# jianzongwu/betrayed-by-captions

Hardware: AMD Instinct MI355X
Metric: images/sec (COCO-shaped 1024x1024, 100 queries, forward-only) (higher is better)
Workload: dtype f32; 1 GPU; configs[1]: R50 + 100 queries, 1024x1024, batch 2/GPU, forward-only; global_batch=2, parallelism=replicas x1, precision=fp32 (parity mode, f16x3 MFMA), hip_graph=True, x3_overflow=False, library_fallbacks=0

## Files before the change

### betrayed-by-captions_amd/csrc/x3s_gemm.hip

```cpp
#include <mutex>
#include "x3.h"

typedef __attribute__((address_space(3))) void* xs_lds_t;

struct XsConv {
  int H, W, C, OH, OW, KW, stride, pad, taps;
};

struct XsArgs {
  const void* A;
  int lda;
  int a_rpb;
  uint32_t a_bstride;
  CggX3W w;
  const float* bias;
  const void* res;
  int ldr, res_fmt, res_mod;
  void* out;
  int ldc, out_fmt;
  int M, N, K, relu, tiles_n, n_tiles32;
  XsConv cv;
  uint32_t a_bytes, w_bytes;
  int* flag;
};

template <int N>
__device__ __forceinline__ void xs_wait_vmcnt() {
  asm volatile("s_waitcnt vmcnt(%0)" ::"n"(N) : "memory");
}

__device__ __forceinline__ void xs_barrier() {
  asm volatile("" ::: "memory");
  __builtin_amdgcn_s_barrier();
  asm volatile("" ::: "memory");
}

#define XS_OOB 0xFFFFFF00u

struct XsTap {
  int c, c0, tap, ky, kx;
};

struct XsEpi {
  __amdgpu_buffer_rsrc_t orsrc, rrsrc;
  float lo_clamp;
  int mr0;
  int pb, y0, x0;
};

__device__ __forceinline__ uint32_t xs_sel(uint32_t a, uint32_t b, uint32_t mask) { return (b & mask) | (a & ~mask); }

__device__ __forceinline__ uint2 xs_pair_swap(const uint2 v) {
  uint2 r;
  r.x = cgg_lane_xor1(v.x);
  r.y = cgg_lane_xor1(v.y);
  return r;
}

__device__ __forceinline__ void xs_load_res(u32x4 (&rv)[4], const XsArgs& p, const __amdgpu_buffer_rsrc_t rrsrc, int& mres, int ncol0,
                                            int lane) {
  const int q = lane & 7;
  const bool cok = ncol0 + 4 * q < p.N;
  const uint32_t coff = (uint32_t)(ncol0 * 4 + 16 * q);
#pragma unroll
  for (int ps = 0; ps < 4; ++ps) {
    int mr = mres + 8 * ps;
    if (p.res_mod) {
      mr = mr >= p.res_mod ? mr - p.res_mod : mr;
      if (p.res_mod < 32) mr %= p.res_mod;
    }
    rv[ps] = __builtin_amdgcn_raw_buffer_load_b128(rrsrc, cok ? (uint32_t)(mr * p.ldr) * 4u + coff : XS_OOB, 0, 0);
  }
  mres += 32;
  if (p.res_mod) mres = p.res_mod >= 32 ? (mres >= p.res_mod ? mres - p.res_mod : mres) : mres % p.res_mod;
}

template <int RES, int OUT, int TW = 0>
__device__ __forceinline__ float xs_finish_column(const float* scratch, int TM_, const XsArgs& p, const XsEpi& e, int mrow0, int ncol0,
                                                  int lane, float amax, const u32x4 (&rv0)[4], bool have_rv0) {
  const int r8 = lane >> 3, q = lane & 7;
  const uint32_t om = 0u - (uint32_t)(q & 1);
  const bool cok = ncol0 + 4 * q < p.N;
  const uint32_t coff = (uint32_t)(ncol0 * 4 + 16 * q);
  int mres = e.mr0;
  auto load_res = [&](u32x4 (&rv)[4]) { xs_load_res(rv, p, e.rrsrc, mres, ncol0, lane); };
  u32x4 rv[4], rn[4];
  if (RES) {
    if (have_rv0) {
#pragma unroll
      for (int ps = 0; ps < 4; ++ps) rv[ps] = rv0[ps];
      mres += 32;
      if (p.res_mod) mres = p.res_mod >= 32 ? (mres >= p.res_mod ? mres - p.res_mod : mres) : mres % p.res_mod;
    } else {
      load_res(rv);
    }
  }
#pragma unroll 1
  for (int mt = 0; mt < TM_; ++mt) {
    const float* sc = scratch + mt * 1024;
    if (RES && mt + 1 < TM_) load_res(rn);
    f32x4 v[4];
#pragma unroll
    for (int ps = 0; ps < 4; ++ps) {
      const int rr = r8 + 8 * ps;
      v[ps] = *reinterpret_cast<const f32x4*>(sc + rr * 32 + (q ^ ((rr >> 1) & 1)) * 4);
    }
#pragma unroll
    for (int ps = 0; ps < 4; ++ps) {
      const int rr = r8 + 8 * ps;
      f32x4 w = v[ps];
      if (RES == 1) {
        w += __builtin_bit_cast(f32x4, rv[ps]) * CGG_X3_ASCALE;
      } else if (RES == 2) {
        const uint32_t r0 = rv[ps][0], r1 = rv[ps][1], r2 = rv[ps][2], r3 = rv[ps][3];
        const uint2 keep = {xs_sel(r0, r2, om), xs_sel(r1, r3, om)};
        const uint2 send = {xs_sel(r2, r0, om), xs_sel(r3, r1, om)};
        const uint2 got = xs_pair_swap(send);
        const uint2 hh = {xs_sel(keep.x, got.x, om), xs_sel(keep.y, got.y, om)};
        const uint2 ll = {xs_sel(got.x, keep.x, om), xs_sel(got.y, keep.y, om)};
        const f32x2 h0 = __builtin_convertvector(__builtin_bit_cast(f16x2, hh.x), f32x2);
        const f32x2 h1 = __builtin_convertvector(__builtin_bit_cast(f16x2, hh.y), f32x2);
        const f32x2 l0 = __builtin_convertvector(__builtin_bit_cast(f16x2, ll.x), f32x2);
        const f32x2 l1 = __builtin_convertvector(__builtin_bit_cast(f16x2, ll.y), f32x2);
        w += f32x4{h0[0] + l0[0], h0[1] + l0[1], h1[0] + l1[0], h1[1] + l1[1]};
      }
#pragma unroll
      for (int k = 0; k < 4; ++k) w[k] = fmaxf(w[k], e.lo_clamp);
      uint32_t oo;
      if constexpr (TW > 0) {
        const int R = mrow0 + 32 * mt + rr, oy = e.y0 + R / TW, ox = e.x0 + R % TW;
        oo = (cok && oy < p.cv.H && ox < p.cv.W) ? (uint32_t)((e.pb + oy * p.cv.W + ox) * p.ldc) * 4u + coff : XS_OOB;
      } else {
        oo = cok ? (uint32_t)((mrow0 + 32 * mt + rr) * p.ldc) * 4u + coff : XS_OOB;
      }
      u32x4 o;
      if (OUT == 2) {
        const float wmax = __builtin_fmaxf(__builtin_fmaxf(fabsf(w[0]), fabsf(w[1])), __builtin_fmaxf(fabsf(w[2]), fabsf(w[3])));
        amax = __builtin_fmaxf(amax, (TW > 0 && oo == XS_OOB) ? 0.f : wmax);
        uint2 h, l;
        cgg_x3_split2(w[0], w[1], h.x, l.x);
        cgg_x3_split2(w[2], w[3], h.y, l.y);
        const uint2 got = xs_pair_swap(uint2{xs_sel(l.x, h.x, om), xs_sel(l.y, h.y, om)});
        o = u32x4{xs_sel(h.x, got.x, om), xs_sel(h.y, got.y, om), xs_sel(got.x, l.x, om), xs_sel(got.y, l.y, om)};
      } else {
        o = __builtin_bit_cast(u32x4, w * CGG_X3_INV_ASCALE);
      }
      __builtin_amdgcn_raw_buffer_store_b128(o, e.orsrc, oo, 0, 0);
    }
    if (RES) {
#pragma unroll
      for (int ps = 0; ps < 4; ++ps) rv[ps] = rn[ps];
    }
  }
  return amax;
}

__device__ __forceinline__ XsEpi xs_epi_setup(const XsArgs& p, int mrow0, int lane) {
  XsEpi e;
  e.orsrc = cgg_buffer_rsrc(p.out, (uint32_t)(((size_t)(p.M - 1) * p.ldc + p.N) * 4));
  const int res_rows = p.res_mod ? p.res_mod : p.M;
  e.rrsrc = cgg_buffer_rsrc(p.res_fmt ? p.res : p.out, p.res_fmt ? (uint32_t)(((size_t)(res_rows - 1) * p.ldr + p.N) * 4) : 0u);
  e.lo_clamp = p.relu ? 0.f : -__builtin_inff();
  e.mr0 = mrow0 + (lane >> 3);
  if (p.res_fmt && p.res_mod) e.mr0 %= p.res_mod;
  return e;
}

template <int TM, int TN, int TW = 0>
__device__ __forceinline__ float xs_epilogue(const f32x16 (&acc)[TM][TN], float* scratch, const XsArgs& p, const XsEpi& e, int mrow0,
                                             int ntile0, int lane, const u32x4 (&rv0)[4]) {
  const int j = lane & 31, hi5 = lane >> 5;
  const int fmt = p.res_fmt * 2 + (p.out_fmt - 1);
  float amax = 0.f;
#pragma unroll
  for (int nt = 0; nt < TN; ++nt) {
    const int ncol = (ntile0 + nt) * 32 + j;
    const bool nok = ncol < p.N;
    const float cs = nok ? p.w.scale[ncol] * CGG_X3_ASCALE : 0.f;
    const float bs = (nok && p.bias) ? p.bias[ncol] * CGG_X3_ASCALE : 0.f;
#pragma unroll
    for (int mt = 0; mt < TM; ++mt) {
#pragma unroll
      for (int r = 0; r < 16; ++r) {
        const int rr = (r & 3) + 8 * (r >> 2) + 4 * hi5;
        scratch[mt * 1024 + rr * 32 + (((j >> 2) ^ ((rr >> 1) & 1)) << 2) + (j & 3)] = acc[mt][nt][r] * cs + bs;
      }
    }
    const int ncol0 = (ntile0 + nt) * 32;
    if constexpr (TW > 0) {
      amax = fmt == 0 ? xs_finish_column<0, 1, TW>(scratch, TM, p, e, mrow0, ncol0, lane, amax, rv0, false)
                      : xs_finish_column<0, 2, TW>(scratch, TM, p, e, mrow0, ncol0, lane, amax, rv0, false);
    } else
    switch (fmt) {
      case 0: amax = xs_finish_column<0, 1>(scratch, TM, p, e, mrow0, ncol0, lane, amax, rv0, false); break;
      case 1: amax = xs_finish_column<0, 2>(scratch, TM, p, e, mrow0, ncol0, lane, amax, rv0, false); break;
      case 2: amax = xs_finish_column<1, 1>(scratch, TM, p, e, mrow0, ncol0, lane, amax, rv0, nt == 0); break;
      case 3: amax = xs_finish_column<1, 2>(scratch, TM, p, e, mrow0, ncol0, lane, amax, rv0, nt == 0); break;
      case 4: amax = xs_finish_column<2, 1>(scratch, TM, p, e, mrow0, ncol0, lane, amax, rv0, nt == 0); break;
      default: amax = xs_finish_column<2, 2>(scratch, TM, p, e, mrow0, ncol0, lane, amax, rv0, nt == 0); break;
    }
  }
  return amax;
}

template <int TM, int TN, int MT>
__device__ __forceinline__ void xs_compute_chunk(f32x16 (&acc)[TM][TN], const unsigned char* ab, const unsigned char* bb,
                                               const int (&aoffs)[2][2]) {
  u32x4 bh[2][TN], bl[2][TN], ah[2], al[2];
#pragma unroll
  for (int nt = 0; nt < TN; ++nt) {
    bh[0][nt] = *reinterpret_cast<const u32x4*>(bb + nt * 4096);
    bl[0][nt] = *reinterpret_cast<const u32x4*>(bb + nt * 4096 + 2048);
  }
  ah[0] = *reinterpret_cast<const u32x4*>(ab + aoffs[0][0]);
  al[0] = *reinterpret_cast<const u32x4*>(ab + aoffs[0][1]);
#pragma unroll
  for (int ks = 0; ks < 2; ++ks) {
#pragma unroll
    for (int mt = 0; mt < TM; ++mt) {
      const int cur = (ks * TM + mt) & 1, nxt = cur ^ 1;
      if (mt + 1 < TM) {
        ah[nxt] = *reinterpret_cast<const u32x4*>(ab + (mt + 1) * MT + aoffs[ks][0]);
        al[nxt] = *reinterpret_cast<const u32x4*>(ab + (mt + 1) * MT + aoffs[ks][1]);
      } else if (ks == 0) {
        ah[nxt] = *reinterpret_cast<const u32x4*>(ab + aoffs[1][0]);
        al[nxt] = *reinterpret_cast<const u32x4*>(ab + aoffs[1][1]);
      }
      if (ks == 0 && mt == (TM > 1 ? TM - 2 : 0)) {
#pragma unroll
        for (int nt = 0; nt < TN; ++nt) {
          bh[1][nt] = *reinterpret_cast<const u32x4*>(bb + nt * 4096 + 1024);
          bl[1][nt] = *reinterpret_cast<const u32x4*>(bb + nt * 4096 + 2048 + 1024);
        }
      }
      __builtin_amdgcn_sched_barrier(0);
#pragma unroll
      for (int nt = 0; nt < TN; ++nt)
        acc[mt][nt] = __builtin_amdgcn_mfma_f32_32x32x16_f16(__builtin_bit_cast(f16x8, al[cur]), __builtin_bit_cast(f16x8, bh[ks][nt]),
                                                             acc[mt][nt], 0, 0, 0);
#pragma unroll
      for (int nt = 0; nt < TN; ++nt)
        acc[mt][nt] = __builtin_amdgcn_mfma_f32_32x32x16_f16(__builtin_bit_cast(f16x8, ah[cur]), __builtin_bit_cast(f16x8, bl[ks][nt]),
                                                             acc[mt][nt], 0, 0, 0);
#pragma unroll
      for (int nt = 0; nt < TN; ++nt)
        acc[mt][nt] = __builtin_amdgcn_mfma_f32_32x32x16_f16(__builtin_bit_cast(f16x8, ah[cur]), __builtin_bit_cast(f16x8, bh[ks][nt]),
                                                             acc[mt][nt], 0, 0, 0);
    }
  }
}

template <bool CONV, int TM, int TN, int WM, int WN, int KG, int SA, int SB>
__global__ __launch_bounds__(64 * WM * WN * KG) void cgg_gemm_x3s_kernel(const XsArgs p) {
  constexpr int NWG = WM * WN, NW = NWG * KG, BM = 32 * TM * WM, BN = 32 * TN * WN;
  constexpr int A_SLOT = KG * BM * 128, B_SLOT = KG * BN * 128;
  constexpr int NA = BM / 8 / NWG, NB = BN / 8 / NWG;
  constexpr int DA = SA - 1, DB = SB - 1;
  constexpr int LDS = SA * A_SLOT + SB * B_SLOT;
  static_assert(BM % (8 * NWG) == 0 && BN % (8 * NWG) == 0, "tile rows / columns must split evenly over the waves' DMA pieces");
  static_assert(SA >= SB && SB >= 2, "A runs at least as far ahead as B");
  static_assert(LDS >= NWG * TM * 4096 + (KG - 1) * NWG * TM * TN * 4096, "LDS: the rings must cover the reduce buffer + epilogue scratch");
  static_assert(KG == 1 || KG == 2, "one or two k-groups");
  constexpr int WAIT = (DA > DB ? NA : 0) + (DB - 1) * (NA + NB);
  extern __shared__ __attribute__((aligned(16))) unsigned char xs_smem[];
  const int tid = threadIdx.x, lane = tid & 63;
  const int wave = __builtin_amdgcn_readfirstlane(tid >> 6);
  const int j = lane & 31, hi5 = lane >> 5;
  const int kg = wave / NWG, wg = wave - kg * NWG;
  const int wm = wg / WN, wn = wg - wm * WN;
  const int bid = cgg_xcd_remap(blockIdx.x, gridDim.x);
  const int tile_m = bid / p.tiles_n, tile_n = bid - tile_m * p.tiles_n;
  const int m0 = tile_m * BM, nt0 = tile_n * (BN / 32);
  const int KS = p.K >> 4, nchunk = p.K >> 5;
  const int niter = (nchunk + KG - 1) / KG;

  const __amdgpu_buffer_rsrc_t arsrc = cgg_buffer_rsrc(p.A, p.a_bytes);
  uint32_t arow[NA];
  uint32_t amask[NA];
  int ag[NA];
#pragma unroll
  for (int i = 0; i < NA; ++i) {
    const int q = wave + NW * i;
    ag[i] = KG == 1 ? 0 : q / (BM / 8);
    const int r = (q - ag[i] * (BM / 8)) * 8 + (lane >> 3);
    const int u = (lane & 7) ^ ((r >> 1) & 7);
    const int m = m0 + r;
    const int mc = m < p.M ? m : p.M - 1;
    if constexpr (CONV) {
      const int ohw = p.cv.OH * p.cv.OW;
      const int b = mc / ohw, rr = mc - b * ohw;
      const int oy = rr / p.cv.OW, ox = rr - oy * p.cv.OW;
      const int iy0 = oy * p.cv.stride - p.cv.pad, ix0 = ox * p.cv.stride - p.cv.pad;
      arow[i] = (uint32_t)(((b * p.cv.H + iy0) * p.cv.W + ix0) * p.cv.C) * 4u + 16u * u;
      uint32_t mk = 0;
      const int KH = p.cv.taps / p.cv.KW;
      for (int ky = 0; ky < KH; ++ky)
        for (int kx = 0; kx < p.cv.KW; ++kx) {
          const int iy = iy0 + ky, ix = ix0 + kx;
          if (iy >= 0 && iy < p.cv.H && ix >= 0 && ix < p.cv.W) mk |= 1u << (ky * p.cv.KW + kx);
        }
      amask[i] = mk;
    } else {
      if (p.a_rpb > 0) {
        const int b = mc / p.a_rpb;
        arow[i] = ((uint32_t)b * p.a_bstride + (uint32_t)(mc - b * p.a_rpb) * (uint32_t)p.lda) * 4u + 16u * u;
      } else {
        arow[i] = (uint32_t)mc * (uint32_t)p.lda * 4u + 16u * u;
      }
      amask[i] = 0;
    }
  }
  const __amdgpu_buffer_rsrc_t brsrc = cgg_buffer_rsrc(p.w.hi, p.w_bytes);
  uint32_t boff[NB];
  int bg[NB];
#pragma unroll
  for (int i = 0; i < NB; ++i) {
    const int q = wave + NW * i;
    bg[i] = KG == 1 ? 0 : q / (BN / 8);
    const int b = q - bg[i] * (BN / 8);
    const int nt = b >> 2, piece = (b >> 1) & 1, ks = b & 1;
    const int ntc = nt0 + nt < p.n_tiles32 ? nt0 + nt : p.n_tiles32 - 1;
    boff[i] = (uint32_t)(((piece * p.n_tiles32 + ntc) * KS + ks) * 64 + lane) * 16u;
  }

  XsTap at[KG];
#pragma unroll
  for (int g = 0; g < KG; ++g) at[g] = {0, 0, 0, 0, 0};
  auto tap_step = [&](XsTap& t) {
    if (t.c + 1 < nchunk) {
      ++t.c;
      if constexpr (CONV) {
        t.c0 += 32;
        if (t.c0 >= p.cv.C) {
          t.c0 = 0;
          ++t.tap;
          if (++t.kx >= p.cv.KW) {
            t.kx = 0;
            ++t.ky;
          }
        }
      }
    }
  };
  if constexpr (KG == 2) tap_step(at[KG - 1]);
  int a_ld = 0, b_ld = 0, b_c = 0;
  auto issue_a = [&]() {
    unsigned char* sbase = xs_smem + a_ld * A_SLOT;
    uint32_t tapoff[KG];
#pragma unroll
    for (int g = 0; g < KG; ++g) tapoff[g] = CONV ? (uint32_t)(((at[g].ky * p.cv.W + at[g].kx) * p.cv.C + at[g].c0) * 4) : 0u;
#pragma unroll
    for (int i = 0; i < NA; ++i) {
      const int g = ag[i];
      const XsTap& t = (KG == 2 && g) ? at[KG - 1] : at[0];
      uint32_t off;
      if constexpr (CONV) off = ((amask[i] >> t.tap) & 1u) ? arow[i] + ((KG == 2 && g) ? tapoff[KG - 1] : tapoff[0]) : XS_OOB;
      else off = arow[i];
      __builtin_amdgcn_raw_ptr_buffer_load_lds(arsrc, (xs_lds_t)(sbase + (wave + NW * i) * 1024), 16, (int)off,
                                               CONV ? 0 : t.c * 128, 0, 0);
    }
#pragma unroll
    for (int g = 0; g < KG; ++g)
#pragma unroll
      for (int k = 0; k < KG; ++k) tap_step(at[g]);
    a_ld = a_ld + 1 == SA ? 0 : a_ld + 1;
  };
  auto issue_b = [&]() {
    unsigned char* sbase = xs_smem + SA * A_SLOT + b_ld * B_SLOT;
#pragma unroll
    for (int i = 0; i < NB; ++i) {
      int c = b_c + bg[i];
      c = c < nchunk ? c : nchunk - 1;
      __builtin_amdgcn_raw_ptr_buffer_load_lds(brsrc, (xs_lds_t)(sbase + (wave + NW * i) * 1024), 16, (int)boff[i], c * 2048, 0, 0);
    }
    b_c = b_c + KG < nchunk ? b_c + KG : b_c;
    b_ld = b_ld + 1 == SB ? 0 : b_ld + 1;
  };

  f32x16 acc[TM][TN];
#pragma unroll
  for (int a = 0; a < TM; ++a)
#pragma unroll
    for (int b = 0; b < TN; ++b)
#pragma unroll
      for (int r = 0; r < 16; ++r) acc[a][b][r] = 0.f;

  const int sw = (j >> 1) & 7;
  const unsigned char* abase = xs_smem + kg * (BM * 128) + (wm * TM * 32 + j) * 128;
  const unsigned char* bbase = xs_smem + SA * A_SLOT + kg * (BN * 128) + wn * TN * 4096 + lane * 16;
  int aoffs[2][2];
#pragma unroll
  for (int ks = 0; ks < 2; ++ks)
#pragma unroll
    for (int pc = 0; pc < 2; ++pc) aoffs[ks][pc] = ((4 * ks + 2 * hi5 + pc) ^ sw) * 16;

#pragma unroll
  for (int t = -DA; t < 0; ++t) {
    if (t + DB >= 0) issue_b();
    issue_a();
  }
  const XsEpi epi = xs_epi_setup(p, m0 + wm * TM * 32, lane);
  u32x4 rv0[4];
  if (p.res_fmt && (KG == 1 || kg == 0)) {
    int mres = epi.mr0;
    xs_load_res(rv0, p, epi.rrsrc, mres, (nt0 + wn * TN) * 32, lane);
  }
  int a_rd = 0, b_rd = 0;
  for (int it = 0; it < niter; ++it) {
    xs_wait_vmcnt<WAIT>();
    xs_barrier();
    issue_b();
    issue_a();
    if (KG == 1 || KG * it + kg < nchunk) xs_compute_chunk<TM, TN, 4096>(acc, abase + a_rd * A_SLOT, bbase + b_rd * B_SLOT, aoffs);
    a_rd = a_rd + 1 == SA ? 0 : a_rd + 1;
    b_rd = b_rd + 1 == SB ? 0 : b_rd + 1;
  }
  xs_wait_vmcnt<0>();
  xs_barrier();

  if constexpr (KG == 2) {
    u32x4* red = reinterpret_cast<u32x4*>(xs_smem) + (size_t)wg * TM * TN * 256 + lane;
    if (kg == 1) {
#pragma unroll
      for (int mt = 0; mt < TM; ++mt)
#pragma unroll
        for (int nt = 0; nt < TN; ++nt)
#pragma unroll
          for (int q = 0; q < 4; ++q)
            red[((mt * TN + nt) * 4 + q) * 64] = __builtin_bit_cast(u32x4, f32x4{acc[mt][nt][4 * q], acc[mt][nt][4 * q + 1],
                                                                                 acc[mt][nt][4 * q + 2], acc[mt][nt][4 * q + 3]});
    }
    __syncthreads();
    if (kg == 1) return;
#pragma unroll
    for (int mt = 0; mt < TM; ++mt)
#pragma unroll
      for (int nt = 0; nt < TN; ++nt)
#pragma unroll
        for (int q = 0; q < 4; ++q) {
          const f32x4 v = __builtin_bit_cast(f32x4, red[((mt * TN + nt) * 4 + q) * 64]);
#pragma unroll
          for (int k = 0; k < 4; ++k) acc[mt][nt][4 * q + k] += v[k];
        }
  }

  float* scratch = reinterpret_cast<float*>(xs_smem + (KG - 1) * NWG * TM * TN * 4096 + wg * (TM * 4096));
  const float amax = xs_epilogue<TM, TN>(acc, scratch, p, epi, m0 + wm * TM * 32, nt0 + wn * TN, lane, rv0);
  if (p.out_fmt == 2 && p.flag && !(amax <= CGG_X3A_MAX)) atomicOr(p.flag, 1);
}

template <int TH, int TW, int CCH, int TM, int TN, int WM, int WN, int SB, int CPI, int KG>
__global__ __launch_bounds__(64 * WM * WN) void cgg_conv3x3_halo_kernel(const XsArgs p) {
  constexpr int NW = WM * WN, BM = 32 * TM * WM, BN = 32 * TN * WN;
  constexpr int P = TW + 2, HP = (TH + 2) * P, HPP = (HP + 7) / 8 * 8, PLANE = HPP * 128;
  constexpr int NAP = CCH * (HPP / 8), NAI = (NAP + NW - 1) / NW;
  constexpr int B_SLOT = CPI * BN * 128, NB = CPI * BN / 8 / NW, DB = SB - 1;
  constexpr int MT = (32 / TW) * P * 128;
  constexpr int NCHUNK = 9 * CCH, NITER = NCHUNK / CPI;
  constexpr int WAIT = (DB - 1) * NB;
  static_assert(TH * TW == BM && (TW == 8 || TW == 16) && TH % (32 / TW) == 0, "patch = the workgroup's rows, whole m-tiles");
  static_assert(BN % (8 * NW) == 0 && SB >= 2, "B pieces split evenly over the waves");
  static_assert(CCH % CPI == 0, "the chunks of an iteration lie inside one filter tap");
  static_assert((CPI == 1 || CPI == 2) && (KG == 1 || KG == 2) && NCHUNK % 2 == 0, "chunk c accumulates into set c % KG");
  static_assert(CCH * PLANE + SB * B_SLOT >= NW * TM * 4096, "LDS: patch + ring must cover the epilogue scratch");
  static_assert(NAI + DB * NB < 64, "vmcnt counts to 63");
  extern __shared__ __attribute__((aligned(16))) unsigned char xs_smem[];
  const int tid = threadIdx.x, lane = tid & 63;
  const int wave = __builtin_amdgcn_readfirstlane(tid >> 6);
  const int j = lane & 31, hi5 = lane >> 5;
  const int wm = wave / WN, wn = wave - wm * WN;
  const int H = p.cv.H, W = p.cv.W;
  const int ptx = (W + TW - 1) / TW, pty = (H + TH - 1) / TH;
  const int bid = cgg_xcd_remap(blockIdx.x, gridDim.x);
  const int tile_m = bid / p.tiles_n, tile_n = bid - tile_m * p.tiles_n;
  const int img = tile_m / (ptx * pty), pr = tile_m - img * (ptx * pty);
  const int py = pr / ptx, px = pr - py * ptx;
  const int y0 = py * TH, x0 = px * TW, nt0 = tile_n * (BN / 32);
  const int KS = p.K >> 4;

  const __amdgpu_buffer_rsrc_t arsrc = cgg_buffer_rsrc(p.A, p.a_bytes);
#pragma unroll
  for (int i = 0; i < NAI; ++i) {
    const int q = wave + NW * i;
    if (q < NAP) {
      const int c = q / (HPP / 8), hp = (q - c * (HPP / 8)) * 8 + (lane >> 3);
      const int ry = hp / P, cx = hp - ry * P;
      const int key = ((cx + (TW == 8 ? 8 * ry : 0)) >> 1) & 7;
      const int iy = y0 - 1 + ry, ix = x0 - 1 + cx;
      const bool ok = hp < HP && iy >= 0 && iy < H && ix >= 0 && ix < W;
      const uint32_t off = ok ? (uint32_t)(((img * H + iy) * W + ix) * (CCH * 32) + c * 32) * 4u + 16u * ((lane & 7) ^ key) : XS_OOB;
      __builtin_amdgcn_raw_ptr_buffer_load_lds(arsrc, (xs_lds_t)(xs_smem + q * 1024), 16, (int)off, 0, 0, 0);
    }
  }
  const __amdgpu_buffer_rsrc_t brsrc = cgg_buffer_rsrc(p.w.hi, p.w_bytes);
  uint32_t boff[NB];
#pragma unroll
  for (int i = 0; i < NB; ++i) {
    const int b = (wave + NW * i) % (BN / 8);
    const int nt = b >> 2, piece = (b >> 1) & 1, ks = b & 1;
    const int ntc = nt0 + nt < p.n_tiles32 ? nt0 + nt : p.n_tiles32 - 1;
    boff[i] = (uint32_t)(((piece * p.n_tiles32 + ntc) * KS + ks) * 64 + lane) * 16u;
  }
  int b_ld = 0, b_c = 0;
  auto issue_b = [&]() {
    unsigned char* sbase = xs_smem + CCH * PLANE + b_ld * B_SLOT;
#pragma unroll
    for (int i = 0; i < NB; ++i)
      __builtin_amdgcn_raw_ptr_buffer_load_lds(brsrc, (xs_lds_t)(sbase + (wave + NW * i) * 1024), 16, (int)boff[i],
                                               (b_c + (wave + NW * i) / (BN / 8)) * 2048, 0, 0);
    b_c = b_c + CPI < NCHUNK ? b_c + CPI : b_c;
    b_ld = b_ld + 1 == SB ? 0 : b_ld + 1;
  };
#pragma unroll
  for (int t = 0; t < DB; ++t) issue_b();

  f32x16 acc[TM][TN], acc1[TM][TN];
#pragma unroll
  for (int a = 0; a < TM; ++a)
#pragma unroll
    for (int b = 0; b < TN; ++b)
#pragma unroll
      for (int r = 0; r < 16; ++r) acc[a][b][r] = acc1[a][b][r] = 0.f;

  const int r0 = wm * TM * 32 + j, dy0 = r0 / TW, dx = r0 - dy0 * TW;
  const unsigned char* abase = xs_smem + (dy0 * P + dx) * 128;
  const unsigned char* bbase = xs_smem + CCH * PLANE + wn * TN * 4096 + lane * 16;

  XsEpi epi = xs_epi_setup(p, 0, lane);
  epi.pb = img * H * W;
  epi.y0 = y0;
  epi.x0 = x0;
  const u32x4 rv0[4] = {};
  int cc = 0, ky = 0, kx = 0, b_rd = 0;
  auto iteration = [&](f32x16 (&ae)[TM][TN], f32x16 (&ao)[TM][TN]) {
    xs_wait_vmcnt<WAIT>();
    xs_barrier();
    issue_b();
    const int key = (((dx + kx) >> 1) + (TW == 8 ? 4 * ((dy0 + ky) & 1) : 0)) & 7;
    int aoffs[2][2];
#pragma unroll
    for (int ks = 0; ks < 2; ++ks)
#pragma unroll
      for (int pc = 0; pc < 2; ++pc) aoffs[ks][pc] = ((4 * ks + 2 * hi5 + pc) ^ key) * 16;
    xs_compute_chunk<TM, TN, MT>(ae, abase + cc * PLANE + (ky * P + kx) * 128, bbase + b_rd * B_SLOT, aoffs);
    if constexpr (CPI == 2)
      xs_compute_chunk<TM, TN, MT>(ao, abase + (cc + 1) * PLANE + (ky * P + kx) * 128, bbase + b_rd * B_SLOT + BN * 128, aoffs);
    b_rd = b_rd + 1 == SB ? 0 : b_rd + 1;
    if ((cc += CPI) == CCH) {
      cc = 0;
      if (++kx == 3) {
        kx = 0;
        ++ky;
      }
    }
  };
  for (int it = 0; it < NITER; it += (KG == 2 && CPI == 1) ? 2 : 1) {
    if constexpr (KG == 1) {
      iteration(acc, acc);
    } else if constexpr (CPI == 2) {
      iteration(acc, acc1);
    } else {
      iteration(acc, acc);
      iteration(acc1, acc1);
    }
  }
  if constexpr (KG == 2) {
#pragma unroll
    for (int a = 0; a < TM; ++a)
#pragma unroll
      for (int b = 0; b < TN; ++b)
#pragma unroll
        for (int r = 0; r < 16; ++r) acc[a][b][r] += acc1[a][b][r];
  }
  xs_wait_vmcnt<0>();
  xs_barrier();

  float* scratch = reinterpret_cast<float*>(xs_smem + wave * (TM * 4096));
  const float amax = xs_epilogue<TM, TN, TW>(acc, scratch, p, epi, wm * TM * 32, nt0 + wn * TN, lane, rv0);
  if (p.out_fmt == 2 && p.flag && !(amax <= CGG_X3A_MAX)) atomicOr(p.flag, 1);
}


static int* g_xs_flag[CGG_MAX_DEVICES] = {nullptr};
static std::once_flag g_xs_once[CGG_MAX_DEVICES];
int* cgg_x3_overflow_flag_ptr() {
  int dev = 0;
  if (hipGetDevice(&dev) != hipSuccess || dev < 0 || dev >= CGG_MAX_DEVICES) return nullptr;
  std::call_once(g_xs_once[dev], [dev] {
    int* q = nullptr;
    if (hipMalloc(&q, 64) != hipSuccess) return;
    if (hipMemset(q, 0, 64) != hipSuccess) { (void)hipFree(q); return; }
    g_xs_flag[dev] = q;
  });
  return g_xs_flag[dev];
}

extern "C" int cgg_init(int device) {
  int prev = 0;
  hipError_t e = hipGetDevice(&prev);
  CGG_REQUIRE(e == hipSuccess, (int)e, "cgg_init: %s", hipGetErrorString(e));
  CGG_REQUIRE(device >= 0 && device < CGG_MAX_DEVICES, CGG_EINVAL, "cgg_init: device %d (0..%d)", device, CGG_MAX_DEVICES - 1);
  e = hipSetDevice(device);
  CGG_REQUIRE(e == hipSuccess, (int)e, "cgg_init: hipSetDevice(%d): %s", device, hipGetErrorString(e));
  int* f = cgg_x3_overflow_flag_ptr();
  (void)hipSetDevice(prev);
  CGG_REQUIRE(f, CGG_EINVAL, "cgg_init: could not create the overflow flag word on device %d", device);
  return CGG_OK;
}

extern "C" int cgg_x3_overflow_check(int reset, int* value_host, cgg_stream_t stream) {
  CGG_REQUIRE(value_host, CGG_EINVAL, "cgg_x3_overflow_check: null pointer");
  int* f = cgg_x3_overflow_flag_ptr();
  CGG_REQUIRE(f, CGG_EINVAL, "cgg_x3_overflow_check: no flag word on this device");
  hipError_t e = hipMemcpyAsync(value_host, f, sizeof(int), hipMemcpyDeviceToHost, (hipStream_t)stream);
  if (e == hipSuccess) e = hipStreamSynchronize((hipStream_t)stream);
  if (e == hipSuccess && reset) e = hipMemsetAsync(f, 0, sizeof(int), (hipStream_t)stream);
  CGG_REQUIRE(e == hipSuccess, (int)e, "cgg_x3_overflow_check: %s", hipGetErrorString(e));
  return CGG_OK;
}

template <bool CONV, int TM, int TN, int WM, int WN, int KG, int SA, int SB>
static int xs_go(const XsArgs& a, hipStream_t stream, const char* who) {
  constexpr int BN = 32 * TN * WN, BM = 32 * TM * WM;
  constexpr int LDS = KG * (SA * BM + SB * BN) * 128;
  CGG_RAISE_LDS((cgg_gemm_x3s_kernel<CONV, TM, TN, WM, WN, KG, SA, SB>), LDS, who);
  XsArgs b = a;
  b.tiles_n = (a.N + BN - 1) / BN;
  const dim3 grid((unsigned)(((a.M + BM - 1) / BM) * b.tiles_n)), block(64 * WM * WN * KG);
  hipLaunchKernelGGL((cgg_gemm_x3s_kernel<CONV, TM, TN, WM, WN, KG, SA, SB>), grid, block, LDS, stream, b);
  return CGG_OK;
}

template <int TH, int TW, int CCH, int TM, int TN, int WM, int WN, int SB, int CPI, int KG>
static int xs_go_halo(const XsArgs& a, hipStream_t stream, const char* who) {
  constexpr int BN = 32 * TN * WN;
  constexpr int LDS = CCH * (((TH + 2) * (TW + 2) + 7) / 8 * 8) * 128 + SB * CPI * BN * 128;
  CGG_RAISE_LDS((cgg_conv3x3_halo_kernel<TH, TW, CCH, TM, TN, WM, WN, SB, CPI, KG>), LDS, who);
  XsArgs b = a;
  b.tiles_n = (a.N + BN - 1) / BN;
  const int images = a.M / (a.cv.H * a.cv.W);
  const long long patches = (long long)images * ((a.cv.H + TH - 1) / TH) * ((a.cv.W + TW - 1) / TW);
  const dim3 grid((unsigned)(patches * b.tiles_n)), block(64 * WM * WN);
  hipLaunchKernelGGL((cgg_conv3x3_halo_kernel<TH, TW, CCH, TM, TN, WM, WN, SB, CPI, KG>), grid, block, LDS, stream, b);
  return CGG_OK;
}

static int xs_launch_halo(const XsArgs& x, hipStream_t stream, const char* who) {
  switch (x.cv.C) {
    case 64: return xs_go_halo<8, 16, 2, 1, 1, 4, 2, 2, 2, 1>(x, stream, who);
    case 128: return xs_go_halo<8, 16, 4, 2, 1, 2, 4, 2, 2, 2>(x, stream, who);
    default: return xs_go_halo<8, 8, 8, 1, 1, 2, 4, 3, 1, 2>(x, stream, who);
  }
}

static bool xs_halo_pays(int C, int N, int M) { return C < 256 || (long long)((M + 63) / 64) * ((N + 127) / 128) <= 256; }

#define XS_CONFIGS(X)                                                                                                              \
  X(0, 4, 2, 2, 4, 1, 3, 2) X(1, 2, 2, 4, 2, 1, 3, 3) X(2, 2, 2, 2, 4, 1, 3, 3) X(3, 2, 2, 2, 2, 1, 4, 4) X(4, 2, 2, 2, 2, 1, 2, 2)   \
  X(5, 1, 2, 2, 2, 1, 4, 4) X(6, 2, 1, 2, 2, 1, 4, 4) X(7, 1, 1, 2, 2, 1, 4, 4) X(8, 4, 1, 2, 2, 1, 3, 3) X(9, 4, 2, 2, 4, 1, 2, 2)   \
  X(10, 2, 2, 2, 2, 2, 2, 2) X(11, 1, 2, 2, 2, 2, 3, 3) X(12, 1, 1, 2, 2, 2, 4, 4) X(13, 1, 1, 2, 2, 1, 2, 2)                      \
  X(14, 2, 1, 2, 2, 1, 2, 2) X(15, 1, 2, 2, 2, 1, 2, 2) X(16, 1, 1, 2, 2, 2, 2, 2) X(17, 1, 2, 2, 2, 2, 2, 2)
#define XS_NCFG 18
#define XS_HALO_CFG 18
static const int xs_bm[XS_NCFG] = {256, 256, 128, 128, 128, 64, 128, 64, 256, 256, 128, 64, 64, 64, 128, 64, 64, 64};
static const int xs_bn[XS_NCFG] = {256, 128, 256, 128, 128, 128, 64, 64, 64, 256, 128, 128, 64, 64, 64, 128, 64, 128};

static int xs_pick(int M, int N, int K, bool has_res) {
  const long long t = (long long)((M + 127) / 128) * ((N + 127) / 128);
  const int w64 = (N + 63) / 64 * 64, w128 = (N + 127) / 128 * 128;
  const bool narrow = N <= 64 || w64 < w128;
  const bool deep = K >= 512;
  if (narrow) {
    if (deep && (long long)((M + 63) / 64) * ((N + 63) / 64) < 512) return 12;
    return (M >= 16384 && K < 256) || N > 64 ? 14 : 13;
  }
  if (t >= 1024) return (K >= 1024 && N % 256 == 0) ? 9 : ((K <= 128 && !has_res) ? 14 : 4);
  if (t >= 512) return (deep && N % 256 == 0) ? 2 : (N >= 512 ? 4 : 14);
  if (t >= 256) return deep ? 10 : 13;
  if (t >= 128) return deep ? 11 : 13;
  return deep ? 12 : 13;
}

static int xs_launch(bool conv, const char* who, const void* a, int lda, const void* w_x3, const float* bias, const void* res, int ldr,
                     int res_fmt, int res_mod, void* out, int ldc, int out_fmt, int M, int N, int K, int relu, const XsConv& cv,
                     cgg_stream_t stream, int a_rpb = 0, int64_t a_bstride = 0, int force_cfg = -1) {
  CGG_REQUIRE(a && w_x3 && out, CGG_EINVAL, "%s: null pointer", who);
  CGG_REQUIRE(a_rpb >= 0 && (a_rpb == 0 || (!conv && a_bstride >= (int64_t)(a_rpb - 1) * lda + K && a_bstride % 8 == 0)), CGG_EINVAL,
              "%s: bad batched A (rows per image %d, image stride %lld)", who, a_rpb, (long long)a_bstride);
  CGG_REQUIRE(M > 0 && N > 0 && K > 0, CGG_EINVAL, "%s: bad sizes", who);
  CGG_REQUIRE(K % 32 == 0, CGG_EUNSUPPORTED, "%s: K=%d must be a multiple of 32", who, K);
  CGG_REQUIRE(N % 8 == 0, CGG_EUNSUPPORTED, "%s: N=%d must be a multiple of 8", who, N);
  CGG_REQUIRE(out_fmt == 1 || out_fmt == 2, CGG_EINVAL, "%s: out_fmt must be 1 (f32) or 2 (x3a)", who);
  CGG_REQUIRE(res_fmt >= 0 && res_fmt <= 2 && (res_fmt == 0) == (res == nullptr), CGG_EINVAL, "%s: res / res_fmt mismatch", who);
  CGG_REQUIRE(cgg_aligned16(a) && cgg_aligned16(w_x3) && cgg_aligned16(out) && cgg_aligned16(res) && (conv || lda % 8 == 0) &&
                  ldc % 8 == 0 && (!res || ldr % 8 == 0),
              CGG_EALIGN, "%s: pointers must be 16-byte aligned, row strides multiples of 8 (lda=%d ldc=%d ldr=%d)", who, lda, ldc, ldr);
  CGG_REQUIRE(!res || ldr >= N, CGG_EINVAL, "%s: ldr=%d < N", who, ldr);
  CGG_REQUIRE(ldc >= N, CGG_EINVAL, "%s: ldc=%d < N", who, ldc);
  CGG_REQUIRE(res_mod >= 0 && (!res_mod || res), CGG_EINVAL, "%s: res_mod without res", who);
  CGG_REQUIRE(!conv || (cv.taps >= 1 && cv.taps <= 32), CGG_EUNSUPPORTED, "%s: at most 32 filter taps", who);
  const uint64_t a_bytes = conv    ? (uint64_t)(M / (cv.OH * cv.OW)) * cv.H * cv.W * cv.C * 4
                           : a_rpb ? ((uint64_t)((M - 1) / a_rpb) * a_bstride + (uint64_t)((M - 1) % a_rpb) * lda + K) * 4
                                   : ((uint64_t)(M - 1) * lda + K) * 4;
  const uint64_t o_bytes = ((uint64_t)(M - 1) * ldc + N) * 4, r_bytes = res ? ((uint64_t)((res_mod ? res_mod : M) - 1) * ldr + N) * 4 : 0;
  CGG_REQUIRE(a_bytes < 0xFFFFFF00ull && o_bytes < 0xFFFFFF00ull && r_bytes < 0xFFFFFF00ull, CGG_EUNSUPPORTED,
              "%s: an operand spans more than 4 GiB (a %llu, out %llu, res %llu bytes)", who, (unsigned long long)a_bytes,
              (unsigned long long)o_bytes, (unsigned long long)r_bytes);
  XsArgs x;
  x.A = a;
  x.lda = lda;
  x.a_rpb = a_rpb;
  x.a_bstride = (uint32_t)a_bstride;
  x.w = cgg_x3_view(w_x3, N, K);
  x.bias = bias;
  x.res = res;
  x.ldr = ldr;
  x.res_fmt = res_fmt;
  x.res_mod = res_mod;
  x.out = out;
  x.ldc = ldc;
  x.out_fmt = out_fmt;
  x.M = M;
  x.N = N;
  x.K = K;
  x.relu = relu;
  x.tiles_n = 0;
  x.n_tiles32 = (N + 31) / 32;
  x.cv = cv;
  x.a_bytes = (uint32_t)a_bytes;
  x.w_bytes = (uint32_t)(2ull * ((N + 31) / 32) * (K / 16) * 64 * 16);
  x.flag = out_fmt == 2 ? cgg_x3_overflow_flag_ptr() : nullptr;
  CGG_REQUIRE(force_cfg <= XS_HALO_CFG, CGG_EINVAL, "%s: tile configuration %d (0 .. %d, or -1 = by shape)", who, force_cfg,
              XS_HALO_CFG);
  const bool halo_ok = conv && cv.taps == 9 && cv.KW == 3 && cv.stride == 1 && cv.pad == 1 && (cv.C == 64 || cv.C == 128 || cv.C == 256) &&
                       !res;
  CGG_REQUIRE(force_cfg != XS_HALO_CFG || halo_ok, CGG_EUNSUPPORTED,
              "%s: tile configuration %d (halo patch) serves 3 x 3 / stride 1 / pad 1 convolutions of 64, 128 or 256 channels without residual",
              who, XS_HALO_CFG);
  const int cfg = force_cfg >= 0 ? force_cfg : (halo_ok && xs_halo_pays(cv.C, N, M)) ? XS_HALO_CFG : xs_pick(M, N, K, res != nullptr);
  if (cfg == XS_HALO_CFG) {
    const int rc = xs_launch_halo(x, (hipStream_t)stream, who);
    if (rc != CGG_OK) return rc;
    CGG_CHECK_LAUNCH(who);
    return CGG_OK;
  }
  int rc = CGG_OK;
#define XS_CASE(ID, TM, TN, WM, WN, KG, SA, SB)                                                 \
  case ID:                                                                                      \
    rc = conv ? xs_go<true, TM, TN, WM, WN, KG, SA, SB>(x, (hipStream_t)stream, who)            \
              : xs_go<false, TM, TN, WM, WN, KG, SA, SB>(x, (hipStream_t)stream, who);          \
    break;
  switch (cfg) { XS_CONFIGS(XS_CASE) }
#undef XS_CASE
  if (rc != CGG_OK) return rc;
  CGG_CHECK_LAUNCH(who);
  return CGG_OK;
}

extern "C" int cgg_gemm_x3s(const void* a_x3a, int lda, const void* w_x3, const float* bias, const void* res, int ldr, int res_fmt,
                            int res_mod, void* out, int ldc, int out_fmt, int M, int N, int K, int relu, cgg_stream_t stream) {
  const XsConv cv = {0, 0, 0, 0, 0, 0, 0, 0, 0};
  CGG_REQUIRE(lda >= K, CGG_EINVAL, "cgg_gemm_x3s: lda=%d < K", lda);
  return xs_launch(false, "cgg_gemm_x3s", a_x3a, lda, w_x3, bias, res, ldr, res_fmt, res_mod, out, ldc, out_fmt, M, N, K, relu, cv,
                   stream);
}

extern "C" int cgg_gemm_x3s_cfg(const void* a_x3a, int lda, const void* w_x3, const float* bias, const void* res, int ldr, int res_fmt,
                                int res_mod, void* out, int ldc, int out_fmt, int M, int N, int K, int relu, int cfg,
                                cgg_stream_t stream) {
  const XsConv cv = {0, 0, 0, 0, 0, 0, 0, 0, 0};
  CGG_REQUIRE(lda >= K, CGG_EINVAL, "cgg_gemm_x3s_cfg: lda=%d < K", lda);
  return xs_launch(false, "cgg_gemm_x3s_cfg", a_x3a, lda, w_x3, bias, res, ldr, res_fmt, res_mod, out, ldc, out_fmt, M, N, K, relu, cv,
                   stream, 0, 0, cfg);
}

extern "C" int cgg_gemm_x3s_batched(const void* a_x3a, int lda, int rows_per_image, int64_t a_bstride, const void* w_x3,
                                    const float* bias, const void* res, int ldr, int res_fmt, int res_mod, void* out, int ldc,
                                    int out_fmt, int M, int N, int K, int relu, cgg_stream_t stream) {
  const XsConv cv = {0, 0, 0, 0, 0, 0, 0, 0, 0};
  CGG_REQUIRE(lda >= K && rows_per_image > 0, CGG_EINVAL, "cgg_gemm_x3s_batched: lda=%d < K or rows_per_image=%d", lda, rows_per_image);
  return xs_launch(false, "cgg_gemm_x3s_batched", a_x3a, lda, w_x3, bias, res, ldr, res_fmt, res_mod, out, ldc, out_fmt, M, N, K, relu,
                   cv, stream, rows_per_image, a_bstride);
}

static int xs_conv(const void* x_x3a, const void* w_x3, const float* bias, const void* res, int res_fmt, void* out, int out_fmt, int B,
                   int H, int W, int C, int N, int KH, int KW, int stride, int pad, int relu, int cfg, cgg_stream_t stream) {
  CGG_REQUIRE(B > 0 && H > 0 && W > 0 && C > 0 && KH > 0 && KW > 0 && stride > 0 && pad >= 0, CGG_EINVAL,
              "cgg_conv_x3s_nhwc: bad sizes");
  CGG_REQUIRE(C % 32 == 0, CGG_EUNSUPPORTED, "cgg_conv_x3s_nhwc: C=%d must be a multiple of 32", C);
  const int OH = (H + 2 * pad - KH) / stride + 1, OW = (W + 2 * pad - KW) / stride + 1;
  CGG_REQUIRE(OH > 0 && OW > 0, CGG_EINVAL, "cgg_conv_x3s_nhwc: empty output");
  if (KH == 1 && KW == 1 && stride == 1 && pad == 0) {
    const XsConv cv0 = {0, 0, 0, 0, 0, 0, 0, 0, 0};
    return xs_launch(false, "cgg_conv_x3s_nhwc", x_x3a, C, w_x3, bias, res, N, res_fmt, 0, out, N, out_fmt, B * H * W, N, C, relu, cv0,
                     stream, 0, 0, cfg);
  }
  const XsConv cv = {H, W, C, OH, OW, KW, stride, pad, KH * KW};
  return xs_launch(true, "cgg_conv_x3s_nhwc", x_x3a, 0, w_x3, bias, res, N, res_fmt, 0, out, N, out_fmt, B * OH * OW, N,
                   KH * KW * C, relu, cv, stream, 0, 0, cfg);
}

extern "C" int cgg_conv_x3s_nhwc(const void* x_x3a, const void* w_x3, const float* bias, const void* res, int res_fmt, void* out,
                                 int out_fmt, int B, int H, int W, int C, int N, int KH, int KW, int stride, int pad, int relu,
                                 cgg_stream_t stream) {
  return xs_conv(x_x3a, w_x3, bias, res, res_fmt, out, out_fmt, B, H, W, C, N, KH, KW, stride, pad, relu, -1, stream);
}
extern "C" int cgg_conv_x3s_nhwc_cfg(const void* x_x3a, const void* w_x3, const float* bias, const void* res, int res_fmt, void* out,
                                     int out_fmt, int B, int H, int W, int C, int N, int KH, int KW, int stride, int pad, int relu,
                                     int cfg, cgg_stream_t stream) {
  return xs_conv(x_x3a, w_x3, bias, res, res_fmt, out, out_fmt, B, H, W, C, N, KH, KW, stride, pad, relu, cfg, stream);
}

__global__ __launch_bounds__(256) void cgg_x3a_convert_kernel(const u32x4* __restrict__ in, u32x4* __restrict__ out, long long ngroups,
                                                             int decode, int* __restrict__ flag) {
  const long long i = (long long)blockIdx.x * 256 + threadIdx.x;
  if (i >= ngroups) return;
  const u32x4 a = in[2 * i], b = in[2 * i + 1];
  if (decode) {
    float f[8];
    cgg_x3a_decode8(a, b, f);
    out[2 * i] = __builtin_bit_cast(u32x4, f32x4{f[0], f[1], f[2], f[3]});
    out[2 * i + 1] = __builtin_bit_cast(u32x4, f32x4{f[4], f[5], f[6], f[7]});
  } else {
    const f32x4 x = __builtin_bit_cast(f32x4, a), y = __builtin_bit_cast(f32x4, b);
    const float f[8] = {x[0], x[1], x[2], x[3], y[0], y[1], y[2], y[3]};
    float amax = 0.f;
#pragma unroll
    for (int k = 0; k < 8; ++k) amax = fmaxf(amax, fabsf(f[k]));
    u32x4 h, l;
    cgg_x3a_encode8(f, h, l);
    out[2 * i] = h;
    out[2 * i + 1] = l;
    if (flag && !(amax * CGG_X3_ASCALE <= CGG_X3A_MAX)) atomicOr(flag, 1);
  }
}

static int xs_convert(const void* in, void* out, int64_t n, int decode, cgg_stream_t stream, const char* who) {
  CGG_REQUIRE(in && out, CGG_EINVAL, "%s: null pointer", who);
  CGG_REQUIRE(n > 0 && n % 8 == 0, CGG_EINVAL, "%s: element count %lld must be a positive multiple of 8", who, (long long)n);
  CGG_REQUIRE(cgg_aligned16(in) && cgg_aligned16(out), CGG_EALIGN, "%s: 16-B alignment", who);
  const long long ng = n / 8;
  hipLaunchKernelGGL(cgg_x3a_convert_kernel, dim3((unsigned)((ng + 255) / 256)), dim3(256), 0, (hipStream_t)stream, (const u32x4*)in,
                     (u32x4*)out, ng, decode, decode ? nullptr : cgg_x3_overflow_flag_ptr());
  CGG_CHECK_LAUNCH(who);
  return CGG_OK;
}

extern "C" int cgg_x3a_encode(const float* x, void* out_x3a, int64_t n, cgg_stream_t stream) {
  return xs_convert(x, out_x3a, n, 0, stream, "cgg_x3a_encode");
}
extern "C" int cgg_x3a_decode(const void* x_x3a, float* out, int64_t n, cgg_stream_t stream) {
  return xs_convert(x_x3a, out, n, 1, stream, "cgg_x3a_decode");
}
```

### betrayed-by-captions_amd/mask2former_head.py

```python
import copy
import os
import json
import warnings

import torch
import torch.distributed as dist
import torch.nn as nn
import torch.nn.functional as F

from . import ops, runtime
from .assigner import get_uncertain_point_coords_with_randomness, point_sample
from .bert_embeddings import BertEmbeddings
from .config import ConfigDict, to_config_dict
from .registry import (HEADS, build_assigner, build_head, build_loss, build_plugin_layer,
                       build_positional_encoding, build_sampler, build_transformer_layer_sequence)

POINT_LOGITS_X3 = os.environ.get('CGG_POINT_LOGITS_X3', '1') != '0'
DEVICE_ASSIGN = os.environ.get('CGG_DEVICE_ASSIGN', '1') != '0'
BOS_TOKEN = 101
EOS_TOKEN = 102


def get_dist_info():
    if dist.is_available() and dist.is_initialized():
# ... 524 lines not shown
                        pooled=[packed[p] if p is not None else None for p in pools], mask_features=None)
        kv16, sizes = enc['kv16'], enc['sizes']
        mf = enc['mf'] if 'mf' in enc else self.pixel_decoder.stream_fpn(*enc['fpn'])
        L = self.num_transformer_feat_level
        layers = self.transformer_decoder.layers
        H4, W4 = int(mf.shape[1]), int(mf.shape[2])
        packed_full, pooled = self._pack_stream(mf, sizes)
        kvs = self._project_kv_levels(kv16)
        return dict(stream=True, kvs=kvs, sizes=sizes, packed_full=packed_full, pooled=pooled, mask_features=None)

    def _project_kv_levels(self, kv16):
        L = self.num_transformer_feat_level
        layers = self.transformer_decoder.layers
        nl = self.num_transformer_decoder_layers
        E = layers[0].attentions[0].embed_dims
        kvs = [None] * nl
        for l in range(min(L, nl)):
            idx = list(range(l, nl, L))
            ws = tuple(layers[i].attentions[0].attn.in_proj_weight for i in idx)
            bs = tuple(layers[i].attentions[0].attn.in_proj_bias for i in idx)
            wk = runtime.derived_cached('kv_levels_wk', ws, lambda: torch.cat([w[E:2 * E] for w in ws], 0).to(torch.bfloat16).contiguous())
            bk = runtime.derived_cached('kv_levels_bk', bs, lambda: torch.cat([b[E:2 * E] for b in bs], 0).to(torch.bfloat16).contiguous())
            wv = runtime.derived_cached('kv_levels_wv', ws, lambda: torch.cat([w[2 * E:] for w in ws], 0).to(torch.bfloat16).contiguous())
            m16, mp16 = kv16[l]
            if E == 256 and m16.is_contiguous() and mp16.is_contiguous():
                wkp = runtime.derived_cached('kv_levels_wkp', ws, lambda: ops.pack_decoder_k_weight(torch.cat([w[E:2 * E] for w in ws], 0)))
                wvp = runtime.derived_cached('kv_levels_wvp', ws, lambda: ops.pack_linear_weight(torch.cat([w[2 * E:] for w in ws], 0)))
                bkf = runtime.derived_cached('kv_levels_bkf', bs, lambda: torch.cat([b[E:2 * E] for b in bs], 0).float().contiguous())
                k_all, vt_all = ops.decoder_kv_proj(m16, mp16, wkp, bkf, wvp)
            else:
                k_all = F.linear(mp16, wk, bk)
                vt_all = torch.matmul(wv, m16.transpose(1, 2))
            for j, i in enumerate(idx):
                kvs[i] = (k_all[:, :, j * E:(j + 1) * E], vt_all[:, j * E:(j + 1) * E, :])
        return kvs

    def _kv_bf16_ok(self):
        layers = self.transformer_decoder.layers
        return (runtime.is_bf16() and not torch.is_grad_enabled() and self.transformer_decoder.post_norm is not None
                and all(l.stream_ready() for l in layers) and self.query_embed.weight.shape[1] % 32 == 0)

    def _kv_tables(self, level_hw, dev):
        w = self.level_embed.weight
        key = (tuple(level_hw), str(dev), w._version, w.data_ptr())
        hit = self.__dict__.get('_kv_table_cache')
        if hit is None or hit[0] != key:
            with torch.no_grad():
                shift = torch.cat([w[i].view(1, -1).expand(h * wd, -1) for i, (h, wd) in enumerate(level_hw)], 0)
                pos = torch.cat([self.decoder_positional_encoding.flat_unpadded(h, wd, dev) for h, wd in level_hw], 0)
                hit = (key, shift.float().contiguous(), pos.float().contiguous())
            self.__dict__['_kv_table_cache'] = hit
        return hit[1], hit[2]

    def _encode(self, feats, defer_tail=False):
        L = self.num_transformer_feat_level
        pd = self.pixel_decoder
        stream = (hasattr(pd, 'stream_ready') and pd.stream_ready(feats) and pd.num_outs >= L
                  and all(isinstance(p, nn.Identity) for p in self.decoder_input_projs))
        mems, poss, sizes, pooled = [], [], [], []
        if stream:
            layers = self.transformer_decoder.layers
            lv = [(int(f.shape[2]), int(f.shape[3])) for f in list(feats)[::-1][:L]]
            kv_fused = (self._kv_bf16_ok() and pd.num_encoder_levels == L and len(feats) == pd.num_input_levels
                        and all(h * w % 4 == 0 and h * w >= 8 for h, w in lv)
                        and all(l.attentions[0].embed_dims // l.attentions[0].num_heads == 32 for l in layers))
            kv16 = None
            if kv_fused:
                mf, memorys, level_hw, kv16 = pd.forward_stream(feats, kv_tables=self._kv_tables,
                                                                defer_fpn=defer_tail == 2)
                if defer_tail == 2:
                    return dict(stream=True, deferred=True, fpn=mf, kv16=kv16, sizes=[level_hw[i] for i in range(L)])
            else:
                mf, memorys, level_hw = pd.forward_stream(feats)
            mask_features = None
            H4, W4 = int(mf.shape[1]), int(mf.shape[2])
            if kv16 is not None and defer_tail:
                return dict(stream=True, deferred=True, mf=mf, kv16=kv16, sizes=[level_hw[i] for i in range(L)])
            for i in range(L):
                sizes.append(level_hw[i])
                if kv16 is None:
                    mems.append(memorys[i] + self.level_embed.weight[i].view(1, 1, -1))
                    poss.append(self.decoder_positional_encoding.flat_unpadded(level_hw[i][0], level_hw[i][1], mf.device))
            packed_full, pooled = self._pack_stream(mf, sizes)
        elif (hasattr(pd, 'stream_ready_x3') and pd.stream_ready_x3(feats) and pd.num_outs >= L
              and all(isinstance(p, nn.Identity) for p in self.decoder_input_projs)
              and self.transformer_decoder.post_norm is not None and self.query_embed.weight.shape[1] % 32 == 0
              and all(l.stream_ready() for l in self.transformer_decoder.layers)):
            if defer_tail and runtime.x3a_enabled():
                mf, memorys, level_hw = pd.forward_stream_x3(feats, defer_fpn=defer_tail == 2)
                return dict(stream=True, deferred=True, x3a=True, memorys=memorys, sizes=[level_hw[i] for i in range(L)],
                            **({'fpn': mf} if defer_tail == 2 else {'mf': mf}))
            fl = list(feats)
            H4, W4 = int(fl[0].shape[2]), int(fl[0].shape[3])
            pools, uniq = self._x3_pools(H4, W4, [(int(f.shape[2]), int(f.shape[3]))
                                                  for f in (fl[pd.num_input_levels - i - 1] for i in range(L))])
            mf, memorys, level_hw = pd.forward_stream_x3(feats, pack_pools=uniq)
            mask_features = None
            x3a_mem = all(ops.is_x3a(m) for m in memorys[:L])
            for i in range(L):
                h, w = level_hw[i]
                sizes.append((h, w))
                if not x3a_mem:
                    mems.append(memorys[i] + self.level_embed.weight[i].view(1, 1, -1))
                    poss.append(self.decoder_positional_encoding.flat_unpadded(h, w, fl[0].device))
            packed = mf if isinstance(mf, dict) else dict(zip(uniq, ops.pack_mask_feature_nhwc_x3(mf, uniq)))
            packed_full, pooled = packed[1], [packed[p] if p is not None else None for p in pools]
            if x3a_mem:
                kvs = self._project_kv_x3a(memorys, sizes)
                return dict(stream=True, kvs=kvs, sizes=sizes, packed_full=packed_full, pooled=pooled, mask_features=None)
        else:
            if runtime.x3_enabled() and not torch.is_grad_enabled() and feats[0].is_cuda:
                runtime.note_fallback('pixel decoder / head', 'stream_ready_x3() is false for this configuration: module path on f32 '
                                      'library GEMMs')
            feats = [ops.x3a_to_f32(f) if ops.is_x3a(f) else f for f in feats]
            feats = [f.float().contiguous() if f.dtype != torch.float32 else f for f in feats]
            mask_features, memorys = pd(feats)
            mask_features = mask_features.contiguous()
            split = not runtime.is_bf16()
            H4, W4 = mask_features.shape[-2:]
            for i in range(L):
                m = self.decoder_input_projs[i](memorys[i])
                h, w = m.shape[-2:]
                sizes.append((int(h), int(w)))
                mems.append((m.flatten(2).transpose(1, 2) + self.level_embed.weight[i].view(1, 1, -1)).contiguous())
                poss.append(self.decoder_positional_encoding.flat_unpadded(int(h), int(w), m.device))
            feat_d = mask_features.detach()
            packed_full = ops.pack_mask_feature(feat_d, 1, split)
            for (h, w) in sizes:
                s = H4 // h
                ok = h * s == H4 and w * s == W4 and s in (2, 4, 8)
                pooled.append(ops.pack_mask_feature(feat_d, s, split) if ok else None)
        layers = self.transformer_decoder.layers
        if self._kv_bf16_ok() and packed_full.lo is None:
            if stream and kv16 is not None:
                kvs = self._project_kv_levels(kv16)
            elif all(h * w % 4 == 0 and h * w >= 8 for h, w in sizes) and \
                    all(l.attentions[0].embed_dims // l.attentions[0].num_heads == 32 for l in layers):
                m16 = [m.to(torch.bfloat16) for m in mems]
                mp16 = [(m + p[None]).to(torch.bfloat16) for m, p in zip(mems, poss)]
                kvs = [layers[i].attentions[0].project_kv_bf16(m16[i % L], mp16[i % L])
                       for i in range(self.num_transformer_decoder_layers)]
            else:
                kvs = [layers[i].attentions[0].project_kv(mems[i % L], poss[i % L])
                       for i in range(self.num_transformer_decoder_layers)]
            return dict(stream=True, kvs=kvs, sizes=sizes, packed_full=packed_full, pooled=pooled, mask_features=None)
        kvs = [layers[i].attentions[0].project_kv(mems[i % L], poss[i % L])
               for i in range(self.num_transformer_decoder_layers)]
        x3_stream = (runtime.x3_enabled() and not torch.is_grad_enabled() and packed_full.hi.is_cuda
                     and self.transformer_decoder.post_norm is not None and all(l.stream_ready() for l in layers)
                     and self.query_embed.weight.shape[1] % 32 == 0)
        return dict(stream=x3_stream, kvs=kvs, sizes=sizes, packed_full=packed_full, pooled=pooled,
                    mask_features=mask_features)

    def _project_kv_x3a(self, memorys, sizes):
        layers = self.transformer_decoder.layers
        L, nl = self.num_transformer_feat_level, self.num_transformer_decoder_layers
        kvs = [None] * nl
        for lvl in range(L):
            idx = list(range(lvl, nl, L))
            attns = [layers[i].attentions[0] for i in idx]
            h, w = sizes[lvl]
            mem = memorys[lvl].as_subclass(torch.Tensor)
            B = mem.shape[0]
            pos = self.decoder_positional_encoding.flat_unpadded(h, w, mem.device)
            E = attns[0].embed_dims

            def make(attns=attns, pos=pos, lvl=lvl, E=E):
                le = self.level_embed.weight[lvl].double()
                ws, tabs = [], []
                for a in attns:
                    w_kv, b_kv = a.kv_weight()
                    wd, bd = w_kv.double(), b_kv.double()
                    kb = (pos.double() + le) @ wd[:E].t() + bd[:E]
                    vb = (le @ wd[E:].t() + bd[E:]).expand(pos.shape[0], E)
                    ws.append(w_kv.float())
                    tabs.append(torch.cat([kb, vb], 1))
                return ops.pack_linear_weight_x3(torch.cat(ws, 0).contiguous()), torch.cat(tabs, 1).float().contiguous()

            params = tuple(p for a in attns for p in (a.attn.in_proj_weight, a.attn.in_proj_bias)) + (self.level_embed.weight, pos)
            wk, table = runtime.derived_cached('kv_stack_x3a', params, make)
            nout = table.shape[1]
            kv_all = ops.gemm_x3s(mem, wk, nout, None, res=table, res_mod=h * w).view(B, h * w, nout)
            for j, i in enumerate(idx):
                kvs[i] = kv_all[:, :, j * 2 * E:(j + 1) * 2 * E]
        return kvs

    def _decode(self, enc, B, all_masks=True):
        if enc.get('deferred'):
            enc = self._finish_encode(enc)
        kvs, sizes, packed_full, pooled = enc['kvs'], enc['sizes'], enc['packed_full'], enc['pooled']
        mask_features = enc['mask_features']
        L = self.num_transformer_feat_level
        layers = self.transformer_decoder.layers
        if enc['stream']:
            return self._decode_stream(B, kvs, sizes, packed_full, pooled, all_masks)
        query_feat = self.query_feat.weight.unsqueeze(0).expand(B, -1, -1)
        query_embed = self.query_embed.weight.unsqueeze(0).expand(B, -1, -1)

        cls_pred_list, cls_emb_pred_list, mask_pred_list = [], [], []
        nl = self.num_transformer_decoder_layers
        cls_pred, cls_emb_pred, mask_pred, bits = self.forward_head(
            query_feat, mask_features, sizes[0], packed_full, pooled[0], want_mask=all_masks or nl == 0)
        cls_pred_list.append(cls_pred)
        cls_emb_pred_list.append(cls_emb_pred)
        mask_pred_list.append(mask_pred)
        for i in range(nl):
            level_idx = i % L
            if self.attn_mask_hook is not None:
                bits = self.attn_mask_hook(i, bits)
            ops.attn_mask_fix_full_rows(bits, sizes[level_idx][0] * sizes[level_idx][1])
            layer = layers[i]
            if tuple(layer.operation_order) == ('cross_attn', 'norm', 'self_attn', 'norm', 'ffn', 'norm'):
                query_feat = layer.forward_fast(query_feat, query_embed, kvs[i], bits)
            else:
                raise NotImplementedError(f'operation_order {layer.operation_order} has no MI355X fast path')
            last = i == nl - 1
            nxt = (i + 1) % L
            cls_pred, cls_emb_pred, mask_pred, bits = self.forward_head(
                query_feat, mask_features, sizes[nxt], packed_full, pooled[nxt],
                want_mask=all_masks or last, want_attn=not last)
            cls_pred_list.append(cls_pred)
            cls_emb_pred_list.append(cls_emb_pred)
            mask_pred_list.append(mask_pred)
        return cls_pred_list, cls_emb_pred_list, mask_pred_list

    def forward(self, feats, img_metas):
        return self._forward(feats, img_metas, all_masks=True)

    def preprocess_gt(self, gt_labels_list, gt_masks_list, gt_semantic_segs, img_metas):
        if gt_semantic_segs is None:
            gt_semantic_segs = [None] * len(gt_labels_list)
        labels_out, masks_out = [], []
        for gt_labels, gt_masks, sem, meta in zip(gt_labels_list, gt_masks_list, gt_semantic_segs, img_metas):
            pad_h, pad_w = meta['pad_shape'][:2]
            if torch.is_tensor(gt_masks):
                tm = gt_masks.to(device=gt_labels.device, dtype=torch.bool)
                dh, dw = pad_h - tm.shape[-2], pad_w - tm.shape[-1]
                if dh or dw:
                    tm = F.pad(tm, (0, dw, 0, dh), value=False)
            else:
                tm = gt_masks.pad((pad_h, pad_w), pad_val=0).to_tensor(dtype=torch.bool, device=gt_labels.device)
            if sem is None:
                labels_out.append(gt_labels)
                masks_out.append(tm.long())
                continue
            sem = sem.squeeze(0)
            stuff_masks, stuff_labels = [], []
            for label in torch.unique(sem, sorted=False):
                if label < self.num_things_classes or label >= self.num_classes:
                    continue
                stuff_masks.append(sem == label)
                stuff_labels.append(label)
            if stuff_masks:
                labels = torch.cat([gt_labels, torch.stack(stuff_labels, 0)], 0)
                masks = torch.cat([tm, torch.stack(stuff_masks, 0)], 0)
            else:
                labels, masks = gt_labels, tm
            labels_out.append(labels)
            masks_out.append(masks.long())
        return labels_out, masks_out

    def _get_cls_emb_logits(self, cls_emb_preds):
        return torch.matmul(cls_emb_preds, self.class_embs.t()) / self.softmax_temperature

    def _rand(self, kind, shape, device):
        if self.point_hook is not None:
            return self.point_hook(kind, shape, device)
        return torch.rand(*shape, device=device)

    def _draw_points(self, device):
        return self._rand('target', (1, self.num_points, 2), device)

    def _target_inputs(self, cls_score, cls_emb_logit, mask_pred, gt_labels, gt_masks):
        num_queries, num_gts = cls_score.shape[0], gt_labels.shape[0]
        point_coords = self._draw_points(cls_score.device)
        mask_points_pred = point_sample(mask_pred.unsqueeze(1), point_coords.repeat(num_queries, 1, 1)).squeeze(1)
        gt_points_masks = point_sample(gt_masks.unsqueeze(1).float(), point_coords.repeat(num_gts, 1, 1)).squeeze(1)
        return (cls_score, cls_emb_logit, mask_points_pred, gt_labels, gt_points_masks)

    def _targets_from_assign(self, assign_result, mask_pred, gt_labels, gt_masks):
        sampling_result = self.sampler.sample(assign_result, mask_pred, gt_masks)
        pos_inds, neg_inds = sampling_result.pos_inds, sampling_result.neg_inds
        labels = gt_labels.new_full((self.num_queries, ), self.num_classes, dtype=torch.long)
        labels[pos_inds] = gt_labels[sampling_result.pos_assigned_gt_inds]
        label_weights = gt_labels.new_ones((self.num_queries, ))
        mask_targets = gt_masks[sampling_result.pos_assigned_gt_inds]
        mask_weights = mask_pred.new_zeros((self.num_queries, ))
        mask_weights[pos_inds] = 1.0
        return labels, label_weights, mask_targets, mask_weights, pos_inds, neg_inds

    def _get_target_single(self, cls_score, cls_emb_logit, mask_pred, gt_labels, gt_masks, img_metas):
        item = self._target_inputs(cls_score, cls_emb_logit, mask_pred, gt_labels, gt_masks)
        assign_result = self.assigner.assign(*item, img_metas)
        return self._targets_from_assign(assign_result, mask_pred, gt_labels, gt_masks)

    def get_targets(self, cls_scores_list, cls_emb_logits_list, mask_preds_list, gt_labels_list,
                    gt_masks_list, img_metas):
        items = [self._target_inputs(c, e, m, gl, gm) for c, e, m, gl, gm in
                 zip(cls_scores_list, cls_emb_logits_list, mask_preds_list, gt_labels_list, gt_masks_list)]
        assigns = self.assigner.assign_batch(items)
        res = [self._targets_from_assign(a, m, gl, gm)
               for a, m, gl, gm in zip(assigns, mask_preds_list, gt_labels_list, gt_masks_list)]
        labels_list, label_weights_list, mask_targets_list, mask_weights_list, pos_l, neg_l = map(list, zip(*res))
        num_total_pos = sum(int(i.numel()) for i in pos_l)
        num_total_neg = sum(int(i.numel()) for i in neg_l)
        return labels_list, label_weights_list, mask_targets_list, mask_weights_list, num_total_pos, num_total_neg

    def _fast_targets_ok(self):
        from .assigner import (ClassificationCost, CrossEntropyLossCost, DiceCost, MaskHungarianAssignerOpen,
                               MaskPseudoSampler)
        a = self.assigner
        return (type(a) is MaskHungarianAssignerOpen and type(self.sampler) is MaskPseudoSampler
                and type(a.cls_cost) is ClassificationCost and type(a.cls_emb_cost) is ClassificationCost
                and type(a.mask_cost) is CrossEntropyLossCost and type(a.dice_cost) is DiceCost)

    def _targets_batched(self, all_cls_scores, emb_logits, all_mask_preds, gt_labels_list, gt_f, overlap=None):
        n, B, Q = len(all_cls_scores), all_cls_scores[0].shape[0], all_cls_scores[0].shape[1]
        dev = all_cls_scores[0].device
        P = self.num_points
        a = self.assigner
        if self.point_hook is None:
            pts = torch.rand((n, B, P, 2), device=dev)
        else:
            pts = torch.stack([torch.cat([self._draw_points(dev) for _ in range(B)], 0) for _ in range(n)], 0)
        with torch.no_grad():
            mf0 = all_mask_preds[0].mask_feature if isinstance(all_mask_preds[0], LazyMasks) else None
            if (mf0 is not None and mf0.is_cuda and mf0.dtype == torch.float32 and mf0.shape[1] % 4 == 0
                    and all(isinstance(m, LazyMasks) and m.mask_feature is mf0 for m in all_mask_preds)):
                nhwc = runtime.handed_nhwc(mf0, allow_grad=True)
                nhwc = nhwc if nhwc is not None else mf0.detach().permute(0, 2, 3, 1).contiguous()
                all_pts = pts.permute(1, 0, 2, 3).reshape(B, n * P, 2)
                pred_pts = torch.empty((n, B, Q, P), dtype=torch.float32, device=dev)
                if POINT_LOGITS_X3 and runtime.x3_enabled() and ops.point_sample_nhwc_x3_ok(nhwc, all_pts, n) \
                        and all(m.mask_embed.shape[-1] == nhwc.shape[-1] and m.mask_embed.shape[1] <= 256 for m in all_mask_preds):
                    packs = ops.point_sample_nhwc_x3(nhwc, all_pts, n)
# ... 544 lines not shown
```

### betrayed-by-captions_amd/ops.py

```python
import ctypes
import os
import math

import torch

from . import _lib
from ._lib import CGG_BF16, CGG_F32, CGG_F32_BF16MFMA, CGG_F32_X3, CONSTANTS, CggError, check, dev_ptr, host_ptr, stream_ptr

_WS_CACHE = {}

KERNEL_EVENTS = None


KERNEL_META = None


class _timed:
    def __init__(self, name, **meta):
        self.name = name
        self.meta = meta
        self.on = KERNEL_EVENTS is not None and not torch.cuda.is_current_stream_capturing()

    def __enter__(self):
        if self.on:
# ... 1426 lines not shown


def nchw_to_nhwc_pad1(x):
    if x.dim() != 4 or x.dtype != torch.float32 or not x.is_cuda:
        raise CggError('nchw_to_nhwc_pad1: (B, C, H, W) float32 ROCm tensor expected')
    B, C, H, W = x.shape
    x = x.contiguous()
    y = zero_border_map(B, H, W, C, x.device)
    _call('cgg_nchw_to_nhwc_pad1_f32', dev_ptr(x), dev_ptr(y), B, C, H, W, stream_ptr(x.device))
    return y


def nhwc_to_nchw(x):
    B, H, W, C = x.shape
    return transpose_f32(x.view(B, H * W, C)).view(B, C, H, W)


def wgrad_x3(dy, x, want_bias=False, amax=None):
    if dy.dim() != 2 or x.dim() != 2 or dy.shape[0] != x.shape[0] or dy.dtype != torch.float32 or x.dtype != torch.float32 \
            or dy.stride(1) != 1 or x.stride(1) != 1:
        raise CggError('wgrad_x3: dy (M, N) and x (M, K) must be float32 matrices with contiguous rows')
    M, N = dy.shape
    K = x.shape[1]
    pdy, px = dev_ptr(dy, 'dy', torch.float32, dense=False), dev_ptr(x, 'x', torch.float32, dense=False)
    nbytes = _lib_().cgg_wgrad_x3_workspace_bytes(M, N, K)
    ws = torch.empty(nbytes // 4, dtype=torch.float32, device=dy.device)
    splits = ctypes.c_int(0)
    wsb = torch.empty((nbytes // (4 * N * K)) * N, dtype=torch.float32, device=dy.device) if want_bias else None
    with _timed('wgrad_x3', flops=2.0 * M * N * K, bytes=4.0 * (M * N + M * K + N * K), shape=(M, N, K)):
        if amax is not None:
            _call('cgg_wgrad_x3_scaled', pdy, dy.stride(0), dev_ptr(amax, 'amax', torch.float32), px, x.stride(0), dev_ptr(ws),
                  dev_ptr(wsb), ctypes.byref(splits), M, N, K, stream_ptr(dy.device))
        elif want_bias:
            _call('cgg_wgrad_bias_x3', pdy, dy.stride(0), px, x.stride(0), dev_ptr(ws), dev_ptr(wsb), ctypes.byref(splits), M, N, K,
                  stream_ptr(dy.device))
        else:
            _call('cgg_wgrad_x3', pdy, dy.stride(0), px, x.stride(0), dev_ptr(ws), ctypes.byref(splits), M, N, K, stream_ptr(dy.device))
    gw = ws.view(splits.value, N, K).sum(0) if splits.value > 1 else ws.view(N, K).clone()
    if want_bias:
        return gw, wsb.view(-1, N)[:splits.value].sum(0)
    return gw


def gemm_x3_split(a, packed, N, col2, bias=None, res_table=None):
    if a.dim() != 2 or a.stride(1) != 1 or a.dtype != torch.float32 or not is_x3(packed):
        raise CggError('gemm_x3_split: a must be a 2-D float32 tensor with a contiguous last dim, packed an x3 image')
    M, K = a.shape
    _x3_check(packed, N, K, 'gemm_x3_split')
    y1 = torch.empty((M, col2), dtype=torch.float32, device=a.device)
    y2 = torch.empty((M, N - col2), dtype=torch.float32, device=a.device)
    if res_table is not None and (res_table.dim() != 2 or res_table.shape[1] != N or not res_table.is_contiguous()
                                  or res_table.dtype != torch.float32):
        raise CggError('gemm_x3_split: res_table must be a contiguous (R, N) float32 tensor')
    with _timed('gemm_x3', flops=2.0 * M * N * K, bytes=4.0 * (M * K + M * N + N * K), shape=(M, N, K)):
        _call('cgg_gemm_x3_ex', dev_ptr(a, 'a', torch.float32, dense=False), a.stride(0), dev_ptr(packed),
              dev_ptr(bias, 'bias', torch.float32), dev_ptr(res_table), N if res_table is not None else 0,
              res_table.shape[0] if res_table is not None else 0, dev_ptr(y1), col2, dev_ptr(y2), N - col2, int(col2), M, N, K, 0,
              stream_ptr(a.device))
    return y1, y2


def gemm_x3_table(a, packed, N, res_table, bias=None, out=None):
    if a.dim() != 2 or a.stride(1) != 1 or a.dtype != torch.float32 or not is_x3(packed):
        raise CggError('gemm_x3_table: a must be a 2-D float32 tensor with a contiguous last dim, packed an x3 image')
    M, K = a.shape
    _x3_check(packed, N, K, 'gemm_x3_table')
    if res_table.dim() != 2 or res_table.shape[1] != N or not res_table.is_contiguous() or res_table.dtype != torch.float32 \
            or M % res_table.shape[0]:
        raise CggError('gemm_x3_table: res_table must be a contiguous (R, N) float32 tensor with R dividing the row count')
    y = out if out is not None else torch.empty((M, N), dtype=torch.float32, device=a.device)
    if y.shape != (M, N) or not y.is_contiguous() or y.dtype != torch.float32:
        raise CggError('gemm_x3_table: bad `out`')
    with _timed('gemm_x3', flops=2.0 * M * N * K, bytes=4.0 * (M * K + M * N + N * K), shape=(M, N, K)):
        _call('cgg_gemm_x3_ex', dev_ptr(a, 'a', torch.float32, dense=False), a.stride(0), dev_ptr(packed),
              dev_ptr(bias, 'bias', torch.float32), dev_ptr(res_table), N, res_table.shape[0], dev_ptr(y), N, None, 0, 0, M, N, K, 0,
              stream_ptr(a.device))
    return y


def conv_x3_nhwc(x, packed, N, kernel, stride=1, pad=0, bias=None, res=None, relu=False, amax=None):
    if x.dim() != 4 or not x.is_contiguous() or x.dtype != torch.float32 or not x.is_cuda or not is_x3(packed):
        raise CggError('conv_x3_nhwc: x must be a contiguous (B, H, W, C) float32 ROCm tensor, packed an x3 image')
    B, H, W, C = x.shape
    KH, KW = (kernel, kernel) if isinstance(kernel, int) else kernel
    OH, OW = (H + 2 * pad - KH) // stride + 1, (W + 2 * pad - KW) // stride + 1
    _x3_check(packed, N, C * KH * KW, 'conv_x3_nhwc')
    y = torch.empty((B, OH, OW, N), dtype=torch.float32, device=x.device)
    if res is not None and (tuple(res.shape) != (B, OH, OW, N) or not res.is_contiguous() or res.dtype != torch.float32):
        raise CggError('conv_x3_nhwc: res must be a contiguous (B, OH, OW, N) float32 tensor')
    with _timed('gemm_x3', flops=2.0 * B * OH * OW * N * C * KH * KW,
                bytes=4.0 * (B * H * W * C + B * OH * OW * N * (2 if res is not None else 1) + N * C * KH * KW),
                shape=(B * OH * OW, N, C * KH * KW)):
        if amax is not None:
            _call('cgg_conv_x3_nhwc_scaled', dev_ptr(x), dev_ptr(amax, 'amax', torch.float32), dev_ptr(packed),
                  dev_ptr(bias, 'bias', torch.float32), dev_ptr(res), dev_ptr(y), B, H, W, C, N, KH, KW, int(stride), int(pad),
                  int(bool(relu)), stream_ptr(x.device))
        else:
            _call('cgg_conv_x3_nhwc', dev_ptr(x), dev_ptr(packed), dev_ptr(bias, 'bias', torch.float32), dev_ptr(res), dev_ptr(y), B, H,
                  W, C, N, KH, KW, int(stride), int(pad), int(bool(relu)), stream_ptr(x.device))
    return y


X3A_F32, X3A_SPLIT = 1, 2


class X3ATensor(torch.Tensor):
    """float32-tagged tensor whose storage holds x3a rows (csrc/x3.h: per 8 channels [8 f16 hi | 8 f16 lo] of 16 x): the marker
    the stream modules hand each other (a ResNet's parity-mode outputs, the encoder memories). Views keep the tag; arithmetic on
    it is meaningless -- `x3a_to_f32` gives the values."""


def is_x3a(t):
    return isinstance(t, X3ATensor)


def as_x3a(t):
    return t.as_subclass(X3ATensor)


def x3a_to_f32(t):
    base = t.as_subclass(torch.Tensor)
    if base.dim() == 4 and base.stride(1) == 1 and not base.is_contiguous():
        return x3a_decode(base.permute(0, 2, 3, 1).contiguous()).permute(0, 3, 1, 2)
    return x3a_decode(base.contiguous())


def x3a_encode(x):
    if x.dtype != torch.float32 or not x.is_cuda or not x.is_contiguous() or x.numel() % 8:
        raise CggError('x3a_encode: contiguous float32 ROCm tensor with numel % 8 == 0 expected')
    y = torch.empty_like(x)
    _call('cgg_x3a_encode', dev_ptr(x), dev_ptr(y), x.numel(), stream_ptr(x.device))
    return y


def x3a_decode(x):
    if x.dtype != torch.float32 or not x.is_cuda or not x.is_contiguous() or x.numel() % 8:
        raise CggError('x3a_decode: contiguous float32-tagged ROCm tensor with numel % 8 == 0 expected')
    y = torch.empty_like(x)
    _call('cgg_x3a_decode', dev_ptr(x), dev_ptr(y), x.numel(), stream_ptr(x.device))
    return y


def x3_overflow_check(device, reset=True):
    v = ctypes.c_int(0)
    with torch.cuda.device(device):
        _call('cgg_x3_overflow_check', int(bool(reset)), ctypes.byref(v), stream_ptr(device))
    return v.value != 0


def _x3s_fmt(split):
    return X3A_SPLIT if split else X3A_F32


def gemm_x3s(a, packed, N, bias=None, res=None, res_split=False, res_mod=0, relu=False, out=None, out_split=False, cfg=-1):
    if a.dim() not in (2, 3) or a.stride(-1) != 1 or a.dtype != torch.float32 or not is_x3(packed):
        raise CggError('gemm_x3s: a must be a 2-D / 3-D float32-tagged tensor with a contiguous last dim, packed an x3 image')
    rpb, bstride = 0, 0
    if a.dim() == 3:
        rpb, bstride = int(a.shape[1]), int(a.stride(0))
        M, K, lda = a.shape[0] * a.shape[1], a.shape[2], int(a.stride(1))
    else:
        (M, K), lda = a.shape, int(a.stride(0))
    _x3_check(packed, N, K, 'gemm_x3s')
    y = out if out is not None else torch.empty((M, N), dtype=torch.float32, device=a.device)
    if y.dim() != 2 or y.stride(1) != 1 or y.shape != (M, N) or y.dtype != torch.float32:
        raise CggError('gemm_x3s: bad `out` view')
    if res is not None and (res.dim() != 2 or res.stride(1) != 1 or res.shape != ((res_mod or M), N) or res.dtype != torch.float32):
        raise CggError('gemm_x3s: bad `res` view')
    with _timed('gemm_x3', flops=2.0 * M * N * K, bytes=4.0 * (M * K + M * N * (2 if res is not None and not res_mod else 1)) +
                4.0 * N * K, shape=(M, N, K)):
        pa = dev_ptr(a, 'a', torch.float32, dense=False)
        rest = (dev_ptr(packed), dev_ptr(bias, 'bias', torch.float32), dev_ptr(res, 'res', torch.float32, dense=False),
                res.stride(0) if res is not None else 0, 0 if res is None else _x3s_fmt(res_split), int(res_mod),
                dev_ptr(y, 'out', torch.float32, dense=False), y.stride(0), _x3s_fmt(out_split), M, N, K, int(bool(relu)))
        if rpb:
            _call('cgg_gemm_x3s_batched', pa, lda, rpb, bstride, *rest, stream_ptr(a.device))
        else:
            _call('cgg_gemm_x3s_cfg', pa, lda, *rest, int(cfg), stream_ptr(a.device))
    return y


def conv_x3s_nhwc(x, packed, N, kernel, stride=1, pad=0, bias=None, res=None, res_split=True, relu=False, out_split=True, cfg=-1):
    if x.dim() != 4 or not x.is_contiguous() or x.dtype != torch.float32 or not x.is_cuda or not is_x3(packed):
        raise CggError('conv_x3s_nhwc: x must be a contiguous (B, H, W, C) float32-tagged ROCm tensor, packed an x3 image')
    B, H, W, C = x.shape
    KH, KW = (kernel, kernel) if isinstance(kernel, int) else kernel
    OH, OW = (H + 2 * pad - KH) // stride + 1, (W + 2 * pad - KW) // stride + 1
    _x3_check(packed, N, C * KH * KW, 'conv_x3s_nhwc')
    y = torch.empty((B, OH, OW, N), dtype=torch.float32, device=x.device)
    if res is not None and (tuple(res.shape) != (B, OH, OW, N) or not res.is_contiguous() or res.dtype != torch.float32):
        raise CggError('conv_x3s_nhwc: res must be a contiguous (B, OH, OW, N) float32-tagged tensor')
    with _timed('gemm_x3', flops=2.0 * B * OH * OW * N * C * KH * KW,
                bytes=4.0 * (B * H * W * C + B * OH * OW * N * (2 if res is not None else 1) + N * C * KH * KW),
                shape=(B * OH * OW, N, C * KH * KW)):
        _call('cgg_conv_x3s_nhwc_cfg', dev_ptr(x), dev_ptr(packed), dev_ptr(bias, 'bias', torch.float32), dev_ptr(res),
              0 if res is None else _x3s_fmt(res_split), dev_ptr(y), _x3s_fmt(out_split), B, H, W, C, N, KH, KW, int(stride), int(pad),
              int(bool(relu)), int(cfg), stream_ptr(x.device))
    return y


def pack_linear_weight(weight):
    N, K = weight.shape
    nbytes = _lib_().cgg_linear_rows_packed_bytes(N, K)
    if nbytes <= 0:
        raise CggError(f'pack_linear_weight: unsupported shape {tuple(weight.shape)} (K % 16)')
    out = torch.empty((nbytes,), dtype=torch.uint8, device=weight.device)
    w = weight.detach().float().contiguous()
    _call('cgg_linear_rows_pack', dev_ptr(w, 'weight', torch.float32), dev_ptr(out), N, K, stream_ptr(weight.device))
    return out


def linear_rows_bf16(x, packed, N, bias=None, res=None, relu_cols=0, ln=None, pos=None, want_pos=False, ksplit=1,
                     out=None):
    if x.dim() != 2 or x.stride(1) != 1 or x.dtype != torch.float32:
        raise CggError('linear_rows_bf16: x must be a 2-D float32 tensor with a contiguous last dim')
    M, K = x.shape
    symbol = _x3_fn('linear_rows', packed)
    if ksplit > 1:
        if out is not None or want_pos or ln is not None or relu_cols:
            raise CggError('linear_rows_bf16: split-K returns (ksplit, M, N) partial planes; no out / ln / pos / relu')
        y = torch.empty((int(ksplit), M, N), dtype=torch.float32, device=x.device)
        _call(symbol, dev_ptr(x, 'x', torch.float32, dense=False), x.stride(0), dev_ptr(packed), dev_ptr(bias, 'bias', torch.float32),
              dev_ptr(res, 'res', torch.float32, dense=False), res.stride(0) if res is not None else 0, dev_ptr(y), N, None, None, 0.0,
              None, 0, None, 0, M, N, K, 0, int(ksplit), None, 0, 0, None, 0, 0, stream_ptr(x.device))
        return y
    y = out if out is not None else torch.empty((M, N), dtype=torch.float32, device=x.device)
    if y.dim() != 2 or y.stride(1) != 1 or y.shape != (M, N) or y.dtype != torch.float32:
        raise CggError('linear_rows_bf16: bad `out` view')
    if res is not None and (res.dim() != 2 or res.stride(1) != 1 or res.shape != (M, N)):
        raise CggError('linear_rows_bf16: bad `res` view')
    yp = torch.empty((M, N), dtype=torch.float32, device=x.device) if want_pos else None
    g, b, eps = ln if ln is not None else (None, None, 0.0)
    _call(symbol, dev_ptr(x, 'x', torch.float32, dense=False), x.stride(0), dev_ptr(packed), dev_ptr(bias, 'bias', torch.float32),
          dev_ptr(res, 'res', torch.float32, dense=False), res.stride(0) if res is not None else 0,
          dev_ptr(y, 'out', torch.float32, dense=False), y.stride(0), dev_ptr(g, 'gamma', torch.float32),
          dev_ptr(b, 'beta', torch.float32), float(eps), dev_ptr(pos, 'pos', torch.float32) if want_pos else None,
          pos.shape[0] if want_pos else 0, dev_ptr(yp), N if want_pos else 0, M, N, K, int(relu_cols), int(ksplit), None, 0, 0, None, 0,
          0, stream_ptr(x.device))
    return (y, yp) if want_pos else y


def linear_rows_bf16_qkv(xqk, xv, packed, bias, E):
    M, K = xqk.shape
    for t in (xqk, xv):
        if t.dim() != 2 or t.stride(1) != 1 or t.dtype != torch.float32 or t.shape != (M, K):
            raise CggError('linear_rows_bf16_qkv: inputs must be matching 2-D float32 tensors')
    if E % 256:
        raise CggError('linear_rows_bf16_qkv: E must be a multiple of 256')
    q = torch.empty((M, E), dtype=torch.float32, device=xqk.device)
    kv = torch.empty((M, 2 * E), dtype=torch.float32, device=xqk.device)
    _call(_x3_fn('linear_rows', packed), dev_ptr(xqk, 'xqk', torch.float32, dense=False), xqk.stride(0), dev_ptr(packed),
          dev_ptr(bias, 'bias', torch.float32), None, 0, dev_ptr(q), E, None, None, 0.0, None, 0, None, 0, M, 3 * E, K, 0, 1,
          dev_ptr(xv, 'xv', torch.float32, dense=False), xv.stride(0), 2 * E, dev_ptr(kv), 2 * E, E, stream_ptr(xqk.device))
    return q, kv


def layernorm_chain(a, norm_a, pos=None, norm_b=None):
    nsum, plane = 1, 0
    if a.dim() == 3:
        if not a.is_contiguous():
            raise CggError('layernorm_chain: partial planes must be contiguous')
        nsum, plane = a.shape[0], a.shape[1] * a.shape[2]
        a = a[0]
    M, N = a.shape
    if a.stride(1) != 1:
        raise CggError('layernorm_chain: last dim must be contiguous')
    y = torch.empty((M, N), dtype=torch.float32, device=a.device)
    yp = torch.empty_like(y) if pos is not None else None
    z = torch.empty_like(y) if norm_b is not None else None
    gb, bb, eb = norm_b if norm_b is not None else (None, None, 0.0)
    _call('cgg_layernorm_chain', dev_ptr(a, 'a', torch.float32, dense=False), a.stride(0), dev_ptr(norm_a[0], 'gamma', torch.float32),
          dev_ptr(norm_a[1], 'beta', torch.float32), float(norm_a[2]), dev_ptr(pos, 'pos', torch.float32),
          pos.shape[0] if pos is not None else 0, dev_ptr(gb, 'gamma_b', torch.float32), dev_ptr(bb, 'beta_b', torch.float32),
          float(eb), dev_ptr(y), dev_ptr(yp), dev_ptr(z), M, N, int(nsum), int(plane), stream_ptr(a.device))
    return y, yp, z


def decoder_mid(core, wo, bo, res, norm, pos=None, qkv=None):
    M, C = core.shape
    for t in (core, res):
        if t.dim() != 2 or t.stride(1) != 1 or t.dtype != torch.float32 or t.shape != (M, C):
            raise CggError('decoder_mid: core / res must be matching (M, C) float32 rows')
    dev = core.device
    x1 = torch.empty((M, C), dtype=torch.float32, device=dev)
    q = kv = None
    wqkv = bqkv = None
    if qkv is not None:
        wqkv, bqkv = qkv
        q = torch.empty((M, C), dtype=torch.float32, device=dev)
        kv = torch.empty((M, 2 * C), dtype=torch.float32, device=dev)
    _call(_x3_fn('decoder_mid', wo, wqkv), dev_ptr(core, 'core', torch.float32, dense=False), core.stride(0), dev_ptr(wo),
          dev_ptr(bo, 'bo', torch.float32), dev_ptr(res, 'res', torch.float32, dense=False), res.stride(0),
          dev_ptr(norm[0], 'gamma', torch.float32), dev_ptr(norm[1], 'beta', torch.float32), float(norm[2]),
          dev_ptr(pos, 'pos', torch.float32), pos.shape[0] if pos is not None else 0, dev_ptr(wqkv),
          dev_ptr(bqkv, 'bqkv', torch.float32), dev_ptr(x1), dev_ptr(q), dev_ptr(kv), M, C, stream_ptr(dev))
    return x1, q, kv


def decoder_ffn(x, w1, b1, w2, b2, F):
    M, C = x.shape
    if x.stride(1) != 1 or x.dtype != torch.float32 or F % 256:
        raise CggError('decoder_ffn: x must be (M, C) float32 rows and F a multiple of 256')
    planes = torch.empty((F // 256, M, C), dtype=torch.float32, device=x.device)
    _call(_x3_fn('decoder_ffn', w1, w2), dev_ptr(x, 'x', torch.float32, dense=False), x.stride(0), dev_ptr(w1),
          dev_ptr(b1, 'b1', torch.float32), dev_ptr(w2), dev_ptr(b2, 'b2', torch.float32), dev_ptr(planes), M, C, int(F),
          stream_ptr(x.device))
    return planes


def self_attn_rows_bf16(q, kv, B, num_heads, scale=None):
    M, E = q.shape
    D = E // num_heads
    if q.stride(1) != 1 or kv.stride(1) != 1 or kv.shape != (M, 2 * E) or q.dtype != torch.float32 or kv.dtype != torch.float32:
        raise CggError('self_attn_rows_bf16: q (M, E) / kv (M, 2E) float32 rows expected')
    out = torch.empty((M, E), dtype=torch.float32, device=q.device)
    _call('cgg_self_attn_rows_bf16', dev_ptr(q, 'q', torch.float32, dense=False), q.stride(0),
          dev_ptr(kv, 'kv', torch.float32, dense=False), kv.stride(0), dev_ptr(out), B, M // B, num_heads, D,
          float(scale if scale is not None else D ** -0.5), stream_ptr(q.device))
    return out


DECODER_TAIL_MAX_PLANES = 8


def decoder_tail(planes, norm_a, pos, norm_b, mlp, qproj=None, want_pos=False):
    if planes.dim() != 3 or not planes.is_contiguous() or planes.dtype != torch.float32:
        raise CggError('decoder_tail: planes must be a contiguous (nsum, M, C) float32 tensor')
    nsum, M, C = planes.shape
    dev = planes.device
    y = torch.empty((M, C), dtype=torch.float32, device=dev)
    yp = torch.empty_like(y) if want_pos else None
# ... 1151 lines not shown
```

### betrayed-by-captions_amd/pixel_decoder.py

```python
import math
import os

import torch
import torch.nn as nn
import torch.nn.functional as F

from . import ops, runtime
from .registry import (ATTENTION, FEEDFORWARD_NETWORK, PLUGIN_LAYERS, POSITIONAL_ENCODING,
                       TRANSFORMER_LAYER, TRANSFORMER_LAYER_SEQUENCE, build_attention,
                       build_feedforward_network, build_positional_encoding,
                       build_transformer_layer, build_transformer_layer_sequence)

FUSED_TAIL = os.environ.get('CGG_FUSED_TAIL', '1') != '0'
FUSED_TRAIN_MSDA = os.environ.get('CGG_FUSED_TRAIN_MSDA', '1') != '0'
FUSED_TRAIN_LN = os.environ.get('CGG_FUSED_TRAIN_LN', '1') != '0'
MERGED_PROJ = os.environ.get('CGG_MERGED_PROJ', '1') != '0' and not os.environ.get('CGG_MSDA_GENERIC')


def build_norm(cfg, num_features):
    cfg = dict(cfg)
    t = cfg.pop('type')
    requires_grad = cfg.pop('requires_grad', True)
    if t == 'GN':
        m = nn.GroupNorm(cfg.pop('num_groups'), num_features, **cfg)
# ... 605 lines not shown
        for f in feats:
            if not (f.is_cuda and f.dtype == torch.bfloat16 and f.dim() == 4
                    and f.permute(0, 2, 3, 1).is_contiguous()):
                return False
        for cm in list(self.input_convs) + list(self.lateral_convs) + list(self.output_convs):
            gn = getattr(cm, cm.norm_name, None) if cm.norm_name else None
            if not isinstance(gn, nn.GroupNorm) or gn.num_channels != 256 or gn.num_groups != 32:
                return False
        if not isinstance(self.output_convs[0].activate, nn.ReLU) or self.input_convs[0].activate is not None:
            return False
        return all(tuple(l.operation_order) == ('self_attn', 'norm', 'ffn', 'norm') and self._stream_ok(l)
                   for l in self.encoder.layers)

    @staticmethod
    def _gemm1x1(x2, conv):
        w = runtime.cast_cached(conv.weight).flatten(1)
        if conv.bias is not None:
            return torch.addmm(runtime.cast_cached(conv.bias), x2, w.t())
        return torch.mm(x2, w.t())

    def forward_stream(self, feats, kv_tables=None, defer_fpn=False):
        B = feats[0].shape[0]
        dev = feats[0].device
        C = 256
        level_hw, level_start, N, pos, ref = self._stream_levels(feats)
        needp = not self._proj_fused(C)
        x16 = torch.empty((B, N, C), dtype=torch.bfloat16, device=dev)
        xp16 = torch.empty((B, N, C), dtype=torch.bfloat16, device=dev) if needp else None
        ws = ops.group_norm_nhwc_workspace(B, int(feats[0].shape[2]) * int(feats[0].shape[3]), 32, dev)
        for i in range(self.num_encoder_levels):
            f = feats[self.num_input_levels - i - 1]
            h, w = level_hw[i]
            cm = self.input_convs[i]
            y = self._gemm1x1(f.permute(0, 2, 3, 1).reshape(B * h * w, f.shape[1]), cm.conv).view(B, h * w, C)
            gn = getattr(cm, cm.norm_name)
            off = level_start[i] * C
            ops.group_norm_nhwc(y, gn.weight, gn.bias, 32, gn.eps, ws, out16=(x16, off, N * C), pos=(pos, off) if needp else None,
                                outp16=(xp16, off, N * C) if needp else None)
        kv16 = None
        if kv_tables is not None:
            src, kv = self._encoder_stream_bf16(None, pos, ref, level_hw, level_start, x16, xp16, kv_tables(level_hw, dev))
            if kv is not None:
                kv16 = [(kv[0][B * s0:B * (s0 + h * w)].view(B, h * w, C), kv[1][B * s0:B * (s0 + h * w)].view(B, h * w, C))
                        for s0, (h, w) in zip(level_start, level_hw)]
        else:
            src = self._encoder_stream_bf16(None, pos, ref, level_hw, level_start, x16, xp16)
        mems = [src[:, s0:s0 + h * w, :] for s0, (h, w) in zip(level_start, level_hw)]
        if defer_fpn:
            fpn_args = (feats[0], src, level_hw[-1], level_start[-1], N)
            return fpn_args, mems, level_hw, kv16
        mf = self.stream_fpn(feats[0], src, level_hw[-1], level_start[-1], N)
        if kv_tables is not None:
            return mf, mems, level_hw, kv16
        return mf, mems, level_hw

    def stream_fpn(self, f, src, last_hw, last_start, N):
        B, dev, C = f.shape[0], f.device, 256
        ws = ops.group_norm_nhwc_workspace(B, int(f.shape[2]) * int(f.shape[3]), 32, dev)
        H4, W4 = int(f.shape[2]), int(f.shape[3])
        lat, outc = self.lateral_convs[0], self.output_convs[0]
        y = self._gemm1x1(f.permute(0, 2, 3, 1).reshape(B * H4 * W4, f.shape[1]), lat.conv).view(B, H4 * W4, C)
        gn = getattr(lat, lat.norm_name)
        z = torch.empty((B, H4, W4, C), dtype=torch.bfloat16, device=dev)
        hl, wl = last_hw
        ops.group_norm_nhwc(y, gn.weight, gn.bias, 32, gn.eps, ws, up=(src, last_start * C, N * C, hl, wl), W=W4,
                            out16=(z, 0, H4 * W4 * C))
        w3 = runtime.cast_cached(outc.conv.weight)
        if not w3.is_contiguous(memory_format=torch.channels_last):
            w3 = w3.contiguous(memory_format=torch.channels_last)
            runtime.cast_cache_replace(outc.conv.weight, w3)
        y = F.conv2d(z.permute(0, 3, 1, 2), w3, None if outc.conv.bias is None else runtime.cast_cached(outc.conv.bias),
                     padding=1)
        y = y.contiguous(memory_format=torch.channels_last).permute(0, 2, 3, 1).reshape(B, H4 * W4, C)
        gn = getattr(outc, outc.norm_name)
        ops.group_norm_nhwc(y, gn.weight, gn.bias, 32, gn.eps, ws, relu=True, out16=(z, 0, H4 * W4 * C))
        return self._gemm1x1(z.view(B * H4 * W4, C), self.mask_feature).view(B, H4, W4, -1)

    def stream_ready_x3(self, feats):
        if not runtime.x3_enabled() or torch.is_grad_enabled():
            return False
        if self.num_input_levels - self.num_encoder_levels != 1 or self.mask_feature.out_channels != 256:
            return False
        for f in feats:
            if not (f.is_cuda and f.dtype == torch.float32 and f.dim() == 4 and f.shape[1] % 32 == 0
                    and (f.permute(0, 2, 3, 1).is_contiguous() or f.is_contiguous())):
                return False
        for cm in list(self.input_convs) + list(self.lateral_convs) + list(self.output_convs):
            gn = getattr(cm, cm.norm_name, None) if cm.norm_name else None
            if not isinstance(gn, nn.GroupNorm) or gn.num_channels != 256 or gn.num_groups != 32:
                return False
        if not isinstance(self.output_convs[0].activate, nn.ReLU) or self.input_convs[0].activate is not None:
            return False
        oc = self.output_convs[0].conv
        if tuple(oc.kernel_size) != (3, 3) or tuple(oc.stride) != (1, 1) or tuple(oc.padding) != (1, 1):
            return False
        for c in [cm.conv for cm in list(self.input_convs) + list(self.lateral_convs)] + [self.mask_feature, oc]:
            if c.groups != 1 or tuple(c.dilation) != (1, 1):
                return False
            if c is not oc and (tuple(c.kernel_size) != (1, 1) or tuple(c.stride) != (1, 1) or tuple(c.padding) != (0, 0)):
                return False
        return all(tuple(l.operation_order) == ('self_attn', 'norm', 'ffn', 'norm') and self._stream_ok(l)
                   and isinstance(l.norms[0], nn.LayerNorm) and l.attentions[0].embed_dims == 256 for l in self.encoder.layers)

    def _encoder_stream_x3(self, src, pos, ref, level_hw, level_start):
        B, N, C = src.shape
        lx = runtime.linear_x3
        x3w = lambda lin: runtime.derived_cached('x3_image', (lin.weight,), lambda: ops.pack_linear_weight_x3(lin.weight))
        srcp = None
        for layer in self.encoder.layers:
            attn = layer.attentions[0]
            H = attn.num_heads
            so, aw = attn.sampling_offsets, attn.attention_weights
            w_cat = runtime.derived_cached('msda_wcat32', (so.weight, aw.weight),
                                           lambda: torch.cat([so.weight, aw.weight], 0).float().contiguous())
            b_cat = runtime.derived_cached('msda_bcat32', (so.bias, aw.bias),
                                           lambda: torch.cat([so.bias, aw.bias], 0).float().contiguous())
            value = lx(src, attn.value_proj.weight, attn.value_proj.bias).view(B, N, H, C // H)
            offs = lx(srcp if srcp is not None else src + pos[None], w_cat, b_cat)
            a = ops.msda_forward_fused(value, level_hw, level_start, offs, ref, attn.num_points)
            n0, n1 = layer.norms
            fc1, fc2 = layer.ffns[0].layers[0][0], layer.ffns[0].layers[1]
            if FUSED_TAIL and fc1.out_features % 256 == 0:
                last = layer is self.encoder.layers[-1]
                src, srcp = ops.encoder_layer_tail_x3(a, src.contiguous(), x3w(attn.output_proj), attn.output_proj.bias,
                                                      (n0.weight, n0.bias, n0.eps), x3w(fc1), fc1.bias, x3w(fc2), fc2.bias,
                                                      (n1.weight, n1.bias, n1.eps), pos=pos,
                                                      want_pos=not last)
                continue
            srcp = None
            y = lx(a, attn.output_proj.weight, attn.output_proj.bias, res=src)
            x1 = ops.add_layernorm_stream(y, None, n0.weight, n0.bias, n0.eps, want_bf16=False)[0]
            h = lx(x1, fc1.weight, fc1.bias, relu=True)
            y = lx(h, fc2.weight, fc2.bias, res=x1)
            src = ops.add_layernorm_stream(y, None, n1.weight, n1.bias, n1.eps, want_bf16=False)[0]
        return src

    def _encoder_stream_x3a(self, src, srcp, pos, ref, level_hw, level_start):
        B, N, C = src.shape
        x3w = lambda lin: runtime.derived_cached('x3_image', (lin.weight,), lambda: ops.pack_linear_weight_x3(lin.weight))
        for layer in self.encoder.layers:
            attn = layer.attentions[0]
            H = attn.num_heads
            so, aw, vp = attn.sampling_offsets, attn.attention_weights, attn.value_proj
            n0, n1 = layer.norms
            fc1, fc2 = layer.ffns[0].layers[0][0], layer.ffns[0].layers[1]
            last = layer is self.encoder.layers[-1]
            n_cat = so.weight.shape[0] + aw.weight.shape[0]
            if self._merged_proj_ok(layer):
                w_all = runtime.derived_cached('msda_wall32', (vp.weight, so.weight, aw.weight),
                                               lambda: torch.cat([vp.weight, so.weight, aw.weight], 0).float().contiguous())
                b_all = runtime.derived_cached('msda_ball32', (vp.bias, so.bias, aw.bias),
                                               lambda: torch.cat([vp.bias, so.bias, aw.bias], 0).float().contiguous())

                tab = self._proj_pos_table(layer, pos, so, aw, tuple(level_hw), N, C, n_cat)
                rows_all = runtime.linear_x3s(src.view(B * N, C), w_all, b_all, res=tab, res_mod=N).view(B, N, C + n_cat)
                a = ops.msda_forward_fused_rows(rows_all, level_hw, level_start, ref, attn.num_points, H, C // H)
                src, srcp = ops.encoder_layer_tail_x3(a, src, x3w(attn.output_proj), attn.output_proj.bias,
                                                      (n0.weight, n0.bias, n0.eps), x3w(fc1), fc1.bias, x3w(fc2), fc2.bias,
                                                      (n1.weight, n1.bias, n1.eps), pos=pos, want_pos=False, x3a=True)
                continue
            w_cat = runtime.derived_cached('msda_wcat32', (so.weight, aw.weight),
                                           lambda: torch.cat([so.weight, aw.weight], 0).float().contiguous())
            b_cat = runtime.derived_cached('msda_bcat32', (so.bias, aw.bias),
                                           lambda: torch.cat([so.bias, aw.bias], 0).float().contiguous())
            if srcp is None:
                raise ops.CggError('encoder stream: mixed merged / split projection layers are not supported')
            value = runtime.linear_x3s(src.view(B * N, C), attn.value_proj.weight, attn.value_proj.bias).view(B, N, H, C // H)
            offs = runtime.linear_x3s(srcp.view(B * N, C), w_cat, b_cat).view(B, N, -1)
            a = ops.msda_forward_fused(value, level_hw, level_start, offs, ref, attn.num_points)
            src, srcp = ops.encoder_layer_tail_x3(a, src, x3w(attn.output_proj), attn.output_proj.bias,
                                                  (n0.weight, n0.bias, n0.eps), x3w(fc1), fc1.bias, x3w(fc2), fc2.bias,
                                                  (n1.weight, n1.bias, n1.eps), pos=pos, want_pos=not last, x3a=True)
        return src

    def _proj_pos_table(self, layer, pos, so, aw, level_hw, N, C, n_cat):
        import collections
        cache = self.__dict__.setdefault('_proj_tables', collections.OrderedDict())
        key = (id(layer), level_hw, str(pos.device))
        ver = (so.weight._version, aw.weight._version, so.weight.data_ptr(), aw.weight.data_ptr(), self.level_encoding.weight._version)
        hit = cache.get(key)
        if hit is not None and hit[0] == ver:
            cache.move_to_end(key)
            return runtime.keepalive(hit[1])
        with torch.no_grad():
            w_cat = torch.cat([so.weight, aw.weight], 0).float().contiguous()
            t = torch.zeros((N, C + n_cat), dtype=torch.float32, device=pos.device)
            t[:, C:] = runtime.linear_x3(pos.float().contiguous(), w_cat)
        cache[key] = (ver, t)
        while len(cache) > 2 * len(self.encoder.layers):
            cache.popitem(last=False)
        return runtime.keepalive(t)

    @staticmethod
    def _merged_proj_ok(layer):
        attn = layer.attentions[0]
        so, aw, vp = attn.sampling_offsets, attn.attention_weights, attn.value_proj
        C, H = vp.weight.shape[1], attn.num_heads
        n_cat = so.weight.shape[0] + aw.weight.shape[0]
        return (MERGED_PROJ and H == 8 and C == 256 and vp.weight.shape[0] == 256 and attn.num_levels == 3 and attn.num_points == 4
                and n_cat == 3 * H * attn.num_levels * attn.num_points and (C + n_cat) % 32 == 0
                and all(m.bias is not None for m in (vp, so, aw)))

    def _forward_stream_x3a(self, feats, defer_fpn=False, pack_pools=None):
        B = feats[0].shape[0]
        dev = feats[0].device
        C = 256
        rows = lambda f: (f if ops.is_x3a(f) else ops.x3a_encode(ops.nchw_to_nhwc(f).contiguous()).permute(0, 3, 1, 2)) \
            .as_subclass(torch.Tensor).permute(0, 2, 3, 1).reshape(-1, f.shape[1])
        level_hw, level_start, N, pos, ref = self._stream_levels(feats)
        src = torch.empty((B, N, C), dtype=torch.float32, device=dev)
        need_srcp = not all(self._merged_proj_ok(l) for l in self.encoder.layers)
        srcp = torch.empty((B, N, C), dtype=torch.float32, device=dev) if need_srcp else None
        ws = ops.group_norm_nhwc_workspace(B, int(feats[0].shape[2]) * int(feats[0].shape[3]), 32, dev)
        for i in range(self.num_encoder_levels):
            f = feats[self.num_input_levels - i - 1]
            h, w = level_hw[i]
            cm = self.input_convs[i]
            y = runtime.linear_x3s(rows(f), cm.conv.weight.flatten(1), cm.conv.bias)
            gn = getattr(cm, cm.norm_name)
            ops.group_norm_nhwc_x3a(y.view(B, h * w, C), gn.weight, gn.bias, 32, gn.eps, ws, out=(src, level_start[i] * C, N * C),
                                    pos=(pos, level_start[i] * C) if need_srcp else None,
                                    outp=(srcp, level_start[i] * C) if need_srcp else None)
        src = self._encoder_stream_x3a(src, srcp, pos, ref, level_hw, level_start)
        mems = [ops.as_x3a(src[:, s0:s0 + h * w, :]) for s0, (h, w) in zip(level_start, level_hw)]
        fpn = (rows(feats[0]), int(feats[0].shape[2]), int(feats[0].shape[3]), src, level_start[-1], N, level_hw[-1], ws, pack_pools)
        if defer_fpn:
            return fpn, mems, level_hw
        return self.stream_fpn_x3a(*fpn), mems, level_hw

    def stream_fpn_x3a(self, frows, H4, W4, src, fine_start, N, fine_hw, ws, pack_pools=None):
        C = 256
        B = src.shape[0]
        lat, outc = self.lateral_convs[0], self.output_convs[0]
        hl, wl = fine_hw
        level_start = [fine_start]
        y = runtime.linear_x3s(frows, lat.conv.weight.flatten(1), lat.conv.bias).view(B, H4 * W4, C)
        gn = getattr(lat, lat.norm_name)
        ops.group_norm_nhwc_x3a(y, gn.weight, gn.bias, 32, gn.eps, ws, out=(y, 0, H4 * W4 * C),
                                up=(src, level_start[-1] * C, N * C, hl, wl), W=W4)
        w3 = runtime.derived_cached('x3_conv_image', (outc.conv.weight,), lambda: ops.pack_conv_weight_x3(outc.conv.weight))
        z = ops.conv_x3s_nhwc(y.view(B, H4, W4, C), w3, C, 3, 1, 1, outc.conv.bias, out_split=False).view(B, H4 * W4, C)
        gn = getattr(outc, outc.norm_name)
        if pack_pools is not None:
            wm = self.mask_feature.weight.flatten(1)
            bm = self.mask_feature.bias.detach() if self.mask_feature.bias is not None else None
            wk = runtime.derived_cached('x3_image', (wm,), lambda: ops.pack_linear_weight_x3(wm))
            head = (z.view(B, H4, W4, C), ws, (gn.weight, gn.bias, gn.eps, gn.num_groups), wk, bm, list(pack_pools))
            if ops.mask_feature_head_x3_ok(*head):
                ops.group_norm_nhwc_stats(z, 32, ws)
                return ops.mask_feature_head_x3(*head)
        ops.group_norm_nhwc_x3a(z, gn.weight, gn.bias, 32, gn.eps, ws, out=(z, 0, H4 * W4 * C), relu=True)
        mf = runtime.linear_x3s(z.view(B * H4 * W4, C), self.mask_feature.weight.flatten(1), self.mask_feature.bias)
        return mf.view(B, H4, W4, -1)

    def forward_stream_x3(self, feats, defer_fpn=False, pack_pools=None):
        if runtime.x3a_enabled():
            return self._forward_stream_x3a(feats, defer_fpn=defer_fpn, pack_pools=pack_pools)
        feats = [ops.x3a_to_f32(f) if ops.is_x3a(f) else f for f in feats]
        B = feats[0].shape[0]
        dev = feats[0].device
        C = 256
        level_hw, level_start, N, pos, ref = self._stream_levels(feats)
        src = torch.empty((B, N, C), dtype=torch.float32, device=dev)
        ws = ops.group_norm_nhwc_workspace(B, int(feats[0].shape[2]) * int(feats[0].shape[3]), 32, dev)
        for i in range(self.num_encoder_levels):
            f = feats[self.num_input_levels - i - 1]
            h, w = level_hw[i]
            cm = self.input_convs[i]
            y = runtime.linear_x3(ops.nchw_to_nhwc(f).reshape(B * h * w, f.shape[1]), cm.conv.weight.flatten(1), cm.conv.bias)
            gn = getattr(cm, cm.norm_name)
            ops.group_norm_nhwc(y.view(B, h * w, C), gn.weight, gn.bias, 32, gn.eps, ws, out32=(src, level_start[i] * C, N * C))
        src = self._encoder_stream_x3(src, pos, ref, level_hw, level_start)
        mems = [src[:, s0:s0 + h * w, :] for s0, (h, w) in zip(level_start, level_hw)]
        f = feats[0]
        H4, W4 = int(f.shape[2]), int(f.shape[3])
        lat, outc = self.lateral_convs[0], self.output_convs[0]
        y = runtime.linear_x3(ops.nchw_to_nhwc(f).reshape(B * H4 * W4, f.shape[1]), lat.conv.weight.flatten(1), lat.conv.bias)
        gn = getattr(lat, lat.norm_name)
        hl, wl = level_hw[-1]
        y = y.view(B, H4 * W4, C)
        ops.group_norm_nhwc(y, gn.weight, gn.bias, 32, gn.eps, ws, up=(src, level_start[-1] * C, N * C, hl, wl), W=W4,
                            out32=(y, 0, H4 * W4 * C))
        w3 = runtime.derived_cached('x3_conv_image', (outc.conv.weight,), lambda: ops.pack_conv_weight_x3(outc.conv.weight))
        z = ops.conv_x3_nhwc(y.view(B, H4, W4, C), w3, C, 3, 1, 1, outc.conv.bias).view(B, H4 * W4, C)
        gn = getattr(outc, outc.norm_name)
        ops.group_norm_nhwc(z, gn.weight, gn.bias, 32, gn.eps, ws, relu=True, out32=(z, 0, H4 * W4 * C))
        mf = runtime.linear_x3(z.view(B * H4 * W4, C), self.mask_feature.weight.flatten(1), self.mask_feature.bias)
        return mf.view(B, H4, W4, -1), mems, level_hw

    def forward(self, feats):
        feats = [ops.x3a_to_f32(f) if ops.is_x3a(f) else f for f in feats]
        B = feats[0].shape[0]
        dev = feats[0].device
        srcs, poss, level_hw = [], [], []
        for i in range(self.num_encoder_levels):
            feat = feats[self.num_input_levels - i - 1]
            h, w = feat.shape[-2:]
            level_hw.append((int(h), int(w)))
            rows = runtime.input_level_x3_train(self.input_convs[i], feat)
            if rows is not None:
                srcs.append(rows)
            else:
                with runtime.autocast():
                    proj = self.input_convs[i](feat)
                srcs.append(proj.float().flatten(2).transpose(1, 2))
            poss.append(self.postional_encoding.flat_unpadded(int(h), int(w), dev)
                        + self.level_encoding.weight[i][None])
        level_start, s = [], 0
        for h, w in level_hw:
            level_start.append(s)
            s += h * w
        src = torch.cat(srcs, 1).contiguous()
        pos = torch.cat(poss, 0)
        ref = self._reference_points(level_hw, dev)
        for layer in self.encoder.layers:
            assert tuple(layer.operation_order) == ('self_attn', 'norm', 'ffn', 'norm'), \
                'MSDeformAttnPixelDecoder fast path expects post-norm (self_attn, norm, ffn, norm) layers'
        if runtime.is_bf16() and not torch.is_grad_enabled() and src.shape[-1] == 256 and \
                all(self._stream_ok(l) for l in self.encoder.layers):
            src = self._encoder_stream_bf16(src, pos, ref, level_hw, level_start)
        else:
            fused_ln = (FUSED_TRAIN_LN and runtime.is_bf16() and torch.is_grad_enabled() and src.is_cuda and src.shape[-1] == 256
                        and all(l.attentions[0].dropout.p == 0 and l.ffns[0].plain_relu_ffn()
                                and isinstance(l.norms[0], nn.LayerNorm) and isinstance(l.norms[1], nn.LayerNorm)
                                for l in self.encoder.layers))
            if fused_ln:
                pos_c = pos.contiguous()
                src16, srcp16 = src.to(torch.bfloat16), (src + pos[None]).to(torch.bfloat16)
                n_layers = len(self.encoder.layers)
                for li, layer in enumerate(self.encoder.layers):
                    attn, ffn = layer.attentions[0], layer.ffns[0]
                    out16 = attn.forward_fused(src, None, ref, level_hw, level_start, add_identity=False, src16=src16,
                                               src_pos16=srcp16)
                    mid, mid16, _ = ops.add_layernorm_train(src, out16, layer.norms[0], want_bf16=True)
                    last = li == n_layers - 1
                    nxt = ops.add_layernorm_train(mid, ffn.forward_bf16_noidentity(mid16), layer.norms[1], pos=pos_c,
                                                  want_bf16=not last, want_pos=not last)
                    src, src16, srcp16 = nxt if not last else (nxt, None, None)
            fused_ln32 = (not fused_ln and FUSED_TRAIN_LN and not runtime.is_bf16() and torch.is_grad_enabled() and src.is_cuda
                          and src.dtype == torch.float32 and src.shape[-1] == 256
                          and all(l.attentions[0].dropout.p == 0 and l.ffns[0].plain_relu_ffn()
                                  and isinstance(l.norms[0], nn.LayerNorm) and isinstance(l.norms[1], nn.LayerNorm)
                                  and ops.add_layernorm_train_ok(src, src, l.norms[0]) and ops.add_layernorm_train_ok(src, src, l.norms[1])
                                  for l in self.encoder.layers))
            for layer in ([] if fused_ln else self.encoder.layers):
                attn = layer.attentions[0]
                if fused_ln32 and FUSED_TRAIN_MSDA and runtime.x3_layer_nodes_ok(layer, src):
                    src = runtime.encoder_layer_x3_train(layer, src, pos, ref, level_hw, level_start)
                    continue
                if fused_ln32:
                    out = attn.forward_fused(src, src + pos[None], ref, level_hw, level_start, add_identity=False)
                    mid = ops.add_layernorm_train(src, out.float(), layer.norms[0])
                    src = ops.add_layernorm_train(mid, layer.ffns[0].forward_noidentity(mid).float(), layer.norms[1])
# ... 22 lines not shown
```

### betrayed-by-captions_amd/runtime.py

```python
import contextlib
import weakref

import torch

_STATE = {'precision': 'fp32'}


def set_precision(p):
    if p not in ('fp32', 'bf16'):
        raise ValueError(f"precision must be 'fp32' or 'bf16', got {p!r}")
    if p == 'fp32' and _STATE['precision'] == 'bf16' and 'cudnn_benchmark' in _STATE:
        torch.backends.cudnn.benchmark = _STATE.pop('cudnn_benchmark')
    if p == 'bf16' and _STATE['precision'] != 'bf16':
        _STATE['cudnn_benchmark'] = torch.backends.cudnn.benchmark
    _STATE['precision'] = p
    if p == 'bf16':
        torch.backends.cudnn.benchmark = True


def precision():
    return _STATE['precision']


def is_bf16():
# ... 662 lines not shown
def x3_fpn_level_ok(pd, x, lo_hw):
    import torch.nn as nn
    bf = is_bf16() and _X3
    if not (_X3_FPN_ROWS and _X3_TRAIN and _X3A and (x3_enabled() or bf) and torch.is_grad_enabled() and x.is_cuda
            and x.dtype in ((torch.float32, torch.bfloat16) if bf else (torch.float32,)) and x.dim() == 4 and len(pd.lateral_convs) == 1):
        return False
    lat, outc, mf = pd.lateral_convs[0], pd.output_convs[0], pd.mask_feature
    gn1 = getattr(lat, lat.norm_name, None) if lat.norm_name else None
    gn2 = getattr(outc, outc.norm_name, None) if outc.norm_name else None
    B, Cin, H, W = x.shape
    C = lat.conv.out_channels
    ok = (isinstance(gn1, nn.GroupNorm) and isinstance(gn2, nn.GroupNorm) and gn1.num_groups * 8 == C == gn2.num_channels
          and gn1.num_groups == gn2.num_groups and 256 % gn1.num_groups == 0 and lat.activate is None and isinstance(outc.activate, nn.ReLU)
          and lat.conv.bias is None and outc.conv.bias is None and tuple(lat.conv.kernel_size) == (1, 1) and tuple(mf.kernel_size) == (1, 1)
          and lat.conv.groups == 1 and mf.groups == 1 and tuple(lat.conv.stride) == (1, 1) and tuple(mf.stride) == (1, 1)
          and tuple(lat.conv.padding) == (0, 0) and tuple(mf.padding) == (0, 0)
          and tuple(lat.conv.dilation) == (1, 1) and tuple(mf.dilation) == (1, 1)
          and _conv3x3_geometry_ok(outc.conv)
          and (bf or x3_train_conv3x3_ok(outc.conv, x.new_empty((B, C, H, W))))
          and Cin % 32 == 0 and C % 32 == 0 and mf.out_channels % 32 == 0 and B * H * W >= X3_TRAIN_ROWS
          and B * H * W * max(Cin, C, mf.out_channels) * 4 < _X3_MAX_BYTES and lo_hw[0] > 0 and lo_hw[1] > 0)
    return bool(ok)


def hand_nhwc(nchw, nhwc):
    nchw._cgg_nhwc = nhwc
    nchw._cgg_nhwc_versions = (nchw._version, nhwc._version)
    return nchw


def handed_nhwc(x, allow_grad=False):
    nh = getattr(x, '_cgg_nhwc', None)
    if nh is None or (x.requires_grad and not allow_grad) or x.dim() != 4 or nh.dtype != torch.float32 or not nh.is_contiguous():
        return None
    B, C, H, W = x.shape
    if tuple(nh.shape) != (B, H, W, C) or getattr(x, '_cgg_nhwc_versions', None) != (x._version, nh._version):
        return None
    return nh


def fpn_level_x3_train(pd, x, lo_rows, lo_hw):
    lat, outc, mf = pd.lateral_convs[0], pd.output_convs[0], pd.mask_feature
    gn1, gn2 = getattr(lat, lat.norm_name), getattr(outc, outc.norm_name)
    B, Cin, H, W = x.shape
    nh = handed_nhwc(x)
    if nh is not None:
        xr = nh.view(B, H * W, Cin)
    else:
        xr = _NchwToRowsFn.apply(x.float())
    cur = _X3LinearFn.apply(xr, lat.conv.weight.flatten(1), None)
    y = _X3FpnLevelFn.apply(cur, lo_rows.float(), gn1.weight, gn1.bias, outc.conv.weight, gn2.weight, gn2.bias, gn1.num_groups, gn1.eps, gn2.eps,
                            (H, W), tuple(lo_hw))
    m = _X3LinearFn.apply(y, mf.weight.flatten(1), mf.bias)
    out = _RowsToNchwFn.apply(m, (H, W))
    return hand_nhwc(out, m.detach().view(B, H, W, m.shape[-1]))


X3_CONV_ROWS = 65536


def _conv3x3_geometry_ok(conv):
    return (tuple(conv.kernel_size) == (3, 3) and tuple(conv.stride) == (1, 1) and tuple(conv.padding) == (1, 1)
            and tuple(conv.dilation) == (1, 1) and conv.groups == 1 and conv.bias is None and conv.in_channels % 32 == 0
            and conv.out_channels % 32 == 0 and getattr(conv, 'padding_mode', 'zeros') == 'zeros')


def x3_train_conv3x3_ok(conv, x):
    return (_X3_TRAIN and _X3A and x3_enabled() and torch.is_grad_enabled() and x.is_cuda and x.dtype == torch.float32 and x.dim() == 4
            and _conv3x3_geometry_ok(conv)
            and x.shape[0] * x.shape[2] * x.shape[3] >= X3_CONV_ROWS and x.shape[2] >= 4 and x.shape[3] >= 4
            and x.shape[0] * (x.shape[2] + 2) * (x.shape[3] + 2) * max(conv.in_channels, conv.out_channels) * 4 < _X3_MAX_BYTES)


def conv3x3_x3_train(x, conv):
    return _X3Conv3x3Fn.apply(x, conv.weight)


_X3_MAX_BYTES = 0xFFFFFF00
X3_TRAIN_ROWS = 8192
_X3_TRAIN = _os.environ.get('CGG_X3_TRAIN', '1') != '0'


def x3_train_linear_ok(x, weight):
    return (_X3_TRAIN and x3_enabled() and torch.is_grad_enabled() and x.is_cuda and x.dtype == torch.float32
            and weight.shape[1] % 32 == 0 and weight.shape[0] % 32 == 0 and x.shape[-1] == weight.shape[1]
            and x.numel() // x.shape[-1] >= X3_TRAIN_ROWS
            and (x.numel() // x.shape[-1]) * max(weight.shape) * 4 < _X3_MAX_BYTES)


X3_TRAIN_ROWS_MODULE = 1024


class ParityLinear(torch.nn.Linear):

    def forward(self, x):
        import torch.nn.functional as F
        w = self.weight
        rows = x.numel() // max(x.shape[-1], 1)
        if (_X3_TRAIN and x3_enabled() and not is_bf16() and torch.is_grad_enabled() and x.is_cuda and x.dtype == torch.float32
                and w.dtype == torch.float32 and w.shape[1] % 32 == 0 and w.shape[0] % 32 == 0 and x.shape[-1] == w.shape[1]
                and rows >= X3_TRAIN_ROWS_MODULE and rows * max(w.shape) * 4 < _X3_MAX_BYTES
                and (x.requires_grad or w.requires_grad)):
            return _X3LinearFn.apply(x, w, self.bias)
        return F.linear(x, w, self.bias)


SPLITK_WGRAD_ROWS = 32768


def linear_bf16_train(x, weight, bias=None):
    import torch.nn.functional as F
    rows = x.numel() // x.shape[-1]
    if rows >= SPLITK_WGRAD_ROWS and weight.requires_grad:
        return _SplitKLinearFn.apply(x, weight, bias)
    with torch.autocast(device_type='cuda', dtype=torch.bfloat16):
        return F.linear(x, weight, bias)


def linear(x, weight, bias=None):
    import torch.nn.functional as F
    if is_bf16() and not (torch.is_grad_enabled() and weight.requires_grad):
        y = F.linear(x.to(torch.bfloat16), cast_cached(weight), cast_cached(bias) if bias is not None else None)
        return y.float()
    if is_bf16():
        return linear_bf16_train(x, weight, bias).float()
    if x3_linear_ok(x, weight):
        return linear_x3(x, weight, bias)
    if x3_train_linear_ok(x, weight):
        return _X3LinearFn.apply(x, weight, bias)
    if x3_enabled() and not torch.is_grad_enabled() and x.is_cuda and x.numel() // max(x.shape[-1], 1) >= 512:
        note_fallback('linear', f'K={weight.shape[1]} (K % 32) / dtype {x.dtype}: f32 library GEMM instead of the x3 kernel')
    return F.linear(x, weight, bias)


FALLBACKS = {}


def note_fallback(kind, detail):
    import logging
    if kind not in FALLBACKS:
        logging.getLogger('cgg_amd').warning('parity mode: %s left the x3 stream -- %s', kind, detail)
    FALLBACKS[kind] = FALLBACKS.get(kind, 0) + 1


def library_fallbacks():
    return sum(FALLBACKS.values())


def x3_linear_ok(x, weight):
    return (x3_enabled() and not torch.is_grad_enabled() and x.is_cuda and x.dtype == torch.float32
            and weight.shape[1] % 32 == 0 and x.shape[-1] == weight.shape[1] and x.numel() // x.shape[-1] >= 512)


def linear_x3s(x, weight, bias=None, res=None, res_split=False, res_mod=0, relu=False, out=None, out_split=False):
    from . import ops
    N, K = weight.shape
    x2 = x if x.dim() <= 3 else x.reshape(-1, K)
    wk = derived_cached('x3_image', (weight,), lambda: ops.pack_linear_weight_x3(weight))
    y = ops.gemm_x3s(x2, wk, N, bias.detach() if bias is not None else None, res=res, res_split=res_split, res_mod=res_mod,
                     relu=relu, out=out.view(-1, N) if out is not None else None, out_split=out_split)
    return out if out is not None else y.view(*x.shape[:-1], N)


def linear_x3(x, weight, bias=None, res=None, relu=False, out=None):
    from . import ops
    N, K = weight.shape
    x2 = x.reshape(-1, K)
    if x2.stride(1) != 1 or x2.stride(0) % 4 or x2.data_ptr() % 16:
        x2 = x2.contiguous()
    wk = derived_cached('x3_image', (weight,), lambda: ops.pack_linear_weight_x3(weight))
    r2 = res.reshape(-1, N) if res is not None else None
    y = ops.gemm_x3(x2, wk, N, bias.detach() if bias is not None else None, res=r2, relu=relu,
                    out=out.view(-1, N) if out is not None else None)
    return out if out is not None else y.view(*x.shape[:-1], N)


_CONST = {}


def const_tensor(values, like):
    key = (tuple(values) if isinstance(values, (list, tuple)) else values, like.dtype, str(like.device))
    t = _CONST.get(key)
    if t is None:
        t = like.new_tensor(values)
        _CONST[key] = t
    return t


_PCACHE = {}


def packed_cached(weights, biases=None):
    from . import ops
    allp = tuple(weights) + tuple(b for b in (biases or ()) if b is not None)
    bases = [t._base if t._base is not None else t for t in allp]
    kind = 'packed' if is_bf16() else 'x3'
    key = tuple(_wkey(t, kind) for t in allp)
    hit = _PCACHE.get(key)
    if hit is not None and all(r() is b for r, b in zip(hit[0], bases)) and \
            hit[1] == tuple(b._version for b in bases) and hit[2].device == weights[0].device:
        return hit[2], hit[3], hit[4]
    if len(_PCACHE) > 4096:
        for k in [k for k, v in _PCACHE.items() if any(r() is None for r in v[0])]:
            del _PCACHE[k]
    w = torch.cat([t.detach().float() for t in weights], 0) if len(weights) > 1 else weights[0].detach().float()
    packed = ops.pack_linear_weight(w.contiguous()) if kind == 'packed' else ops.pack_linear_weight_x3(w.contiguous())
    bias = None
    if biases is not None:
        bias = torch.cat([b.detach().float() for b in biases], 0).contiguous() if len(biases) > 1 \
            else biases[0].detach().float().contiguous()
    _PCACHE[key] = ([weakref.ref(b) for b in bases], tuple(b._version for b in bases), packed, bias, int(w.shape[0]))
    return packed, bias, int(w.shape[0])


_DCACHE = {}


_KEEPALIVE = []


class keepalive_scope:

    def __enter__(self):
        self.refs = {}
        _KEEPALIVE.append(self.refs)
        return self.refs

    def __exit__(self, *exc):
        _KEEPALIVE[:] = [r for r in _KEEPALIVE if r is not self.refs]
        return False


def keepalive(val):
    if _KEEPALIVE:
        for refs in _KEEPALIVE:
            refs[id(val)] = val
    return val


def derived_cached(tag, tensors, fn):
    bases = [t._base if t._base is not None else t for t in tensors]
    key = (tag,) + tuple(_wkey(t, None) for t in tensors)
    hit = _DCACHE.get(key)
    if hit is not None and all(r() is b for r, b in zip(hit[0], bases)) and hit[1] == tuple(b._version for b in bases):
        return keepalive(hit[2])
    if len(_DCACHE) > 256:
        for k in [k for k, v in _DCACHE.items() if any(r() is None for r in v[0])]:
            del _DCACHE[k]
    with torch.no_grad():
        val = fn()
    _DCACHE[key] = ([weakref.ref(b) for b in bases], tuple(b._version for b in bases), val)
    return keepalive(val)
```

### include/cgg_hip.h

```cpp
#ifndef CGG_HIP_H_
#define CGG_HIP_H_

#include <stdint.h>

#ifdef __cplusplus
extern "C" {
#endif

#define CGG_VERSION 100

#define CGG_OK 0
#define CGG_EINVAL (-1)
#define CGG_EUNSUPPORTED (-2)
#define CGG_EALIGN (-3)
#define CGG_ELIBRARY (-4)

#define CGG_F32 0
#define CGG_BF16 1
#define CGG_F32_BF16MFMA 2
#define CGG_F32_X3 3

typedef void* cgg_stream_t;

int cgg_version(void);
// ... 76 lines not shown
int cgg_attn_mask_fix_full_rows(uint32_t* bits, int rows, int npix, cgg_stream_t stream);

int cgg_attn_mask_from_logits(const float* logits, uint32_t* bits, int N, int H, int W, int h,
                              int w, cgg_stream_t stream);

int64_t cgg_masked_xattn_workspace_bytes(int B, int Q, int H, int D, int S);
int cgg_masked_xattn_forward(const float* q, const void* kv, const uint32_t* bits, float* out,
                             void* ws, int B, int Q, int H, int D, int S, float scale,
                             int kv_dtype, cgg_stream_t stream);
int cgg_masked_xattn_forward_strided(const float* q, const float* kv, int ldkv, int64_t kv_bstride, const uint32_t* bits,
                                     float* out, void* ws, int B, int Q, int H, int D, int S, float scale, cgg_stream_t stream);
int cgg_masked_xattn_forward_x3(const float* q, const float* kv, int ldkv, int64_t kv_bstride, const uint32_t* bits, float* out,
                                void* ws, int B, int Q, int H, int D, int S, float scale, cgg_stream_t stream);
int cgg_masked_xattn_forward_bf16(const float* q, const void* k, const void* vt, const uint32_t* bits, float* out,
                                  void* ws, int B, int Q, int H, int D, int S, float scale, int ldk, int64_t vt_bstride,
                                  int auto_unmask, cgg_stream_t stream);

int cgg_masked_xattn_forward_lse(const float* q, const void* kv, const uint32_t* bits, float* out, float* lse,
                                 void* ws, int B, int Q, int H, int D, int S, float scale, int kv_dtype,
                                 cgg_stream_t stream);
int64_t cgg_masked_xattn_backward_workspace_bytes(int B, int Q, int H, int D, int S);
int cgg_masked_xattn_backward(const float* q, const void* kv, const uint32_t* bits, const float* out,
                              const float* lse, const float* grad_out, float* grad_q, void* grad_kv, void* ws,
                              int B, int Q, int H, int D, int S, float scale, int kv_dtype, cgg_stream_t stream);
int cgg_masked_xattn_backward_x3(const float* q, const void* kv, const uint32_t* bits, const float* out, const float* lse,
                                 const float* grad_out, const float* grad_out_amax, float* grad_q, void* grad_kv, void* ws, int B,
                                 int Q, int H, int D, int S, float scale, cgg_stream_t stream);

int cgg_window_attn_forward(const float* qkv, const float* table, float* out, float* lse, int B, int Hp, int Wp, int C,
                            int heads, int ws, int shift, float scale, cgg_stream_t stream);
int64_t cgg_window_attn_backward_workspace_bytes(int B, int Hp, int Wp, int heads, int ws);
int cgg_window_attn_backward(const float* qkv, const float* table, const float* lse, const float* grad_out, float* grad_qkv,
                             float* grad_table, void* ws_buf, int B, int Hp, int Wp, int C, int heads, int ws, int shift,
                             float scale, cgg_stream_t stream);

int cgg_grounding_pair_costs(const float* pred, const float* cap, const int32_t* cap_mask, float* cost, int Bp, int Bc,
                             int Q, int T, int d, float inv_temperature, cgg_stream_t stream);
int cgg_grounding_pair_costs_backward(const float* pred, const float* cap, const int32_t* cap_mask,
                                      const float* grad_cost, float* dsim, int Bp, int Bc, int Q, int T, int d,
                                      float inv_temperature, cgg_stream_t stream);

int cgg_ce_rows_forward(const void* logits, const int64_t* target, float* loss, float* lse, int M, int N, int64_t ld,
                        int64_t ignore_index, int dtype, cgg_stream_t stream);
int cgg_ce_rows_backward(void* logits, const int64_t* target, const float* lse, const float* grad_rows, int M, int N,
                         int64_t ld, int64_t ignore_index, int dtype, cgg_stream_t stream);

int cgg_match_cost_rows(const float* x, float* sig, float* sp_sum, float* sig_sum, int rows, int P, int square,
                        cgg_stream_t stream);

int64_t cgg_rle_encode_bitmasks(const uint8_t* bits, int n, int H, int W, int64_t mask_stride_bytes, int row_bytes,
                                int threads, uint8_t* out, int64_t out_cap, int64_t* offsets);

int64_t cgg_rle_transitions_workspace_bytes(int n, int H, int W);
int cgg_rle_transitions(const uint8_t* bits, int n, int H, int W, int64_t mask_stride_bytes, int row_bytes, void* ws,
                        uint32_t* positions, int64_t capacity, int64_t* offsets, cgg_stream_t stream);

int64_t cgg_rle_strings_from_transitions(const uint32_t* positions, const int64_t* offsets, int n, int H, int W,
                                         uint8_t* out, int64_t out_cap, int64_t* out_offsets);
int64_t cgg_rle_encode_colmajor(const uint64_t* cols, int n, int H, int W, int threads, uint8_t* out, int64_t out_cap,
                                int64_t* out_offsets);

int cgg_paint_instances_u8(const uint8_t* img, uint8_t* out, int H, int W, const uint8_t* bits, int n, int64_t mask_stride_bytes,
                           int row_bytes, const uint8_t* keep, const uint8_t* colors, const int32_t* boxes,
                           const uint8_t* box_colors, double alpha, double one_minus_alpha, int thickness, int edges,
                           cgg_stream_t stream);
int cgg_pack_bool_rows_u8(const uint8_t* masks, int64_t rows, int W, int row_bytes, uint8_t* bits, cgg_stream_t stream);
int64_t cgg_label_components_workspace_bytes(int H, int W);
int cgg_label_components_i32(const int32_t* pan, int H, int W, int void_id, void* ws, int64_t* records, int capacity,
                             int32_t* status, cgg_stream_t stream);
int cgg_paint_panoptic_u8(const uint8_t* img, uint8_t* out, const int32_t* pan, int H, int W, const int32_t* ids,
                          const uint8_t* colors, int nids, double alpha, double one_minus_alpha, int edges, cgg_stream_t stream);

int cgg_self_attn_rows_bf16(const float* q, int ldq, const float* kv, int ldkv, float* out, int B, int Q, int H, int D,
                            float scale, cgg_stream_t stream);

int cgg_linear_rows(const float* x, int ldx, const float* w, const float* bias, const float* res, int ldr,
                    float* y, int ldy, int M, int N, int K, int relu, int split, cgg_stream_t stream);
int cgg_add_layernorm(const float* a, const float* b, const float* gamma, const float* beta, float* y,
                      int rows, int N, float eps, cgg_stream_t stream);

int64_t cgg_linear_rows_packed_bytes(int N, int K);
int cgg_linear_rows_pack(const float* w, void* packed, int N, int K, cgg_stream_t stream);
int cgg_linear_rows_bf16(const float* x, int ldx, const void* w_packed, const float* bias, const float* res,
                         int ldr, float* y, int ldy, const float* ln_gamma, const float* ln_beta, float ln_eps,
                         const float* pos, int pos_rows, float* yp, int ldyp, int M, int N, int K, int relu_cols,
                         int ksplit, const float* x2, int ldx2, int x2_col, float* y2, int ldy2, int y2_col,
                         cgg_stream_t stream);

int cgg_layernorm_chain(const float* a, int lda, const float* gamma_a, const float* beta_a, float eps_a,
                        const float* pos, int pos_rows, const float* gamma_b, const float* beta_b, float eps_b,
                        float* y, float* yp, float* z, int rows, int N, int nsum, int64_t plane,
                        cgg_stream_t stream);

int cgg_decoder_tail_bf16(const float* planes, int nsum, int64_t plane_stride, int ld, const float* gamma_a,
                          const float* beta_a, float eps_a, const float* pos, int pos_rows, const float* gamma_b,
                          const float* beta_b, float eps_b, const void* w1, const float* b1, const void* w2,
                          const float* b2, const void* w3, const float* b3, const void* wq, const float* bq, float* y,
                          float* yp, float* mask_embed, float* qn, int M, int C, cgg_stream_t stream);

int cgg_decoder_mid_bf16(const float* core, int ldc, const void* wo, const float* bo, const float* res, int ldr,
                         const float* gamma, const float* beta, float eps, const float* pos, int pos_rows,
                         const void* wqkv, const float* bqkv, float* x1, float* q, float* kv, int M, int C,
                         cgg_stream_t stream);

int cgg_decoder_ffn_bf16(const float* x, int ldx, const void* w1, const float* b1, const void* w2, const float* b2,
                         float* planes, int M, int C, int F, cgg_stream_t stream);

int64_t cgg_x3_packed_bytes(int N, int K);
int cgg_x3_pack(const float* w, void* packed, int N, int K, cgg_stream_t stream);
int cgg_linear_rows_x3(const float* x, int ldx, const void* w_x3, const float* bias, const float* res,
                       int ldr, float* y, int ldy, const float* ln_gamma, const float* ln_beta, float ln_eps,
                       const float* pos, int pos_rows, float* yp, int ldyp, int M, int N, int K, int relu_cols,
                       int ksplit, const float* x2, int ldx2, int x2_col, float* y2, int ldy2, int y2_col,
                       cgg_stream_t stream);
int cgg_decoder_tail_x3(const float* planes, int nsum, int64_t plane_stride, int ld, const float* gamma_a,
                        const float* beta_a, float eps_a, const float* pos, int pos_rows, const float* gamma_b,
                        const float* beta_b, float eps_b, const void* w1, const float* b1, const void* w2,
                        const float* b2, const void* w3, const float* b3, const void* wq, const float* bq, float* y,
                        float* yp, float* mask_embed, float* qn, int M, int C, cgg_stream_t stream);
int cgg_decoder_mid_x3(const float* core, int ldc, const void* wo, const float* bo, const float* res, int ldr,
                       const float* gamma, const float* beta, float eps, const float* pos, int pos_rows,
                       const void* wqkv, const float* bqkv, float* x1, float* q, float* kv, int M, int C,
                       cgg_stream_t stream);
int cgg_decoder_ffn_x3(const float* x, int ldx, const void* w1, const float* b1, const void* w2, const float* b2,
                       float* planes, int M, int C, int F, cgg_stream_t stream);

int cgg_group_norm_nhwc_f32(const float* x, const float* gamma, const float* beta, void* ws, int B, int HW, int C, int groups,
                            float eps, int relu, const float* up_src, int up_h, int up_w, int64_t up_bstride, int W,
                            float* y32, int64_t y32_bstride, void* y16, const float* pos, void* yp16, int64_t y16_bstride,
                            cgg_stream_t stream);
int cgg_pack_mask_feature_nhwc_f32_x3(const float* feat, void* const* hi_host, void* const* lo_host, const int* pools_host,
                                      int n, int B, int C, int H, int W, cgg_stream_t stream);
int cgg_point_sample_nhwc_x3(const float* feat, const float* pts, void* hi, void* lo, int B, int H, int W, int C, int P_total,
                             int P_group, cgg_stream_t stream);
int cgg_encoder_layer_tail_x3(const float* a32, const float* x32, const void* wo_x3, const float* bo, const float* gamma0,
                              const float* beta0, float eps0, const void* w1_x3, const float* b1, const void* w2_x3,
                              const float* b2, const float* gamma1, const float* beta1, float eps1, const float* pos,
                              int pos_rows, float* y32, float* yp32, int M, int C, int F, cgg_stream_t stream);
int cgg_gemm_x3(const float* a, int lda, const void* w_x3, const float* bias, const float* res, int ldr, float* out, int ldc,
                int M, int N, int K, int relu, cgg_stream_t stream);
int cgg_stem_conv7x7_x3_nchw(const float* img, const void* w_packed, const float* wscale, float* out, int B, int H, int W,
                             cgg_stream_t stream);
int cgg_bias_relu_maxpool_nhwc_f32(const float* x, const float* bias, float* y, int B, int H, int W, int C, cgg_stream_t stream);
int cgg_gemm_x3_ex(const float* a, int lda, const void* w_x3, const float* bias, const float* res, int ldr, int res_mod, float* out,
                   int ldc, float* out2, int ldc2, int col2, int M, int N, int K, int relu, cgg_stream_t stream);
int cgg_conv_x3_nhwc(const float* x, const void* w_x3, const float* bias, const float* res, float* out, int B, int H, int W,
                     int C, int N, int KH, int KW, int stride, int pad, int relu, cgg_stream_t stream);

int cgg_gemm_x3s(const void* a_x3a, int lda, const void* w_x3, const float* bias, const void* res, int ldr, int res_fmt,
                 int res_mod, void* out, int ldc, int out_fmt, int M, int N, int K, int relu, cgg_stream_t stream);
int cgg_gemm_x3s_batched(const void* a_x3a, int lda, int rows_per_image, int64_t a_bstride, const void* w_x3, const float* bias,
                         const void* res, int ldr, int res_fmt, int res_mod, void* out, int ldc, int out_fmt, int M, int N, int K,
                         int relu, cgg_stream_t stream);
int cgg_conv_x3s_nhwc(const void* x_x3a, const void* w_x3, const float* bias, const void* res, int res_fmt, void* out,
                      int out_fmt, int B, int H, int W, int C, int N, int KH, int KW, int stride, int pad, int relu,
                      cgg_stream_t stream);
int cgg_x3a_encode(const float* x, void* out_x3a, int64_t n, cgg_stream_t stream);
int cgg_x3a_decode(const void* x_x3a, float* out, int64_t n, cgg_stream_t stream);
int cgg_x3_overflow_check(int reset, int* value_host, cgg_stream_t stream);
int cgg_gemm_x3s_cfg(const void* a_x3a, int lda, const void* w_x3, const float* bias, const void* res, int ldr, int res_fmt,
                     int res_mod, void* out, int ldc, int out_fmt, int M, int N, int K, int relu, int cfg, cgg_stream_t stream);
int cgg_conv_x3s_nhwc_cfg(const void* x_x3a, const void* w_x3, const float* bias, const void* res, int res_fmt, void* out,
                          int out_fmt, int B, int H, int W, int C, int N, int KH, int KW, int stride, int pad, int relu, int cfg,
                          cgg_stream_t stream);
int cgg_bias_relu_maxpool_nhwc_f32_x3a(const float* x, const float* bias, void* y_x3a, int B, int H, int W, int C,
                                       cgg_stream_t stream);
int cgg_group_norm_nhwc_f32_x3a(const float* x, const float* gamma, const float* beta, void* ws, int B, int HW, int C, int groups,
                                float eps, int relu, const void* up_src_x3a, int up_h, int up_w, int64_t up_bstride, int W,
                                void* y_x3a, int64_t y_bstride, const float* pos, void* yp_x3a, cgg_stream_t stream);

int64_t cgg_group_norm_nhwc_backward_workspace_bytes(int B, int HW, int groups);
int cgg_group_norm_nhwc_f32_backward(const float* x, const float* y, const float* dy, const float* stats, const float* gamma, void* ws,
                                     int B, int HW, int C, int groups, float eps, int relu, float* dx, float* tot, float* dlo, int lo_h,
                                     int lo_w, int W, int dx_padded, cgg_stream_t stream);
int cgg_group_norm_nhwc_f32_padout(const float* x, const float* gamma, const float* beta, void* ws, int B, int HW, int C, int groups,
                                   float eps, int relu, const float* up_src, int up_h, int up_w, int64_t up_bstride, int W,
                                   float* y_padded, cgg_stream_t stream);
int cgg_encoder_layer_tail_x3a(const float* a32, const void* x_x3a, const void* wo_x3, const float* bo, const float* gamma0,
                               const float* beta0, float eps0, const void* w1_x3, const float* b1, const void* w2_x3,
                               const float* b2, const float* gamma1, const float* beta1, float eps1, const float* pos,
                               int pos_rows, void* y_x3a, void* yp_x3a, int M, int C, int F, cgg_stream_t stream);
int cgg_group_norm_nhwc_f32_stats(const float* x, void* ws, int B, int HW, int C, int groups, cgg_stream_t stream);
int cgg_mask_feature_head_x3(const float* z, const void* gn_ws, const float* gamma, const float* beta, float eps, int groups,
                             const void* w_x3, const float* bias, void* const* hi_host, void* const* lo_host, const int* pools_host,
                             int n, float* mf, int B, int H, int W, int C, int N, cgg_stream_t stream);
int cgg_mask_feature_head_x3_cfg(const float* z, const void* gn_ws, const float* gamma, const float* beta, float eps, int groups,
                                 const void* w_x3, const float* bias, void* const* hi_host, void* const* lo_host,
                                 const int* pools_host, int n, float* mf, int B, int H, int W, int C, int N, int cfg,
                                 cgg_stream_t stream);

#define CGG_IMAGE_PREP_MAX_DIM 65535
int cgg_image_prep_u8(const uint8_t* staged, int64_t staged_bytes, int64_t table_offset, const int32_t* table_host, int B,
                      const float* mean, const float* std, const float* pad_val, int to_rgb, int pad_before_norm, float* out, int Hb,
                      int Wb, cgg_stream_t stream);

int cgg_train_prep_u8(const uint8_t* staged, int64_t staged_bytes, int64_t img_table_offset, int64_t inst_table_offset,
                      const int32_t* img_table_host, const int32_t* inst_table_host, int B, int N, const float* mean, const float* std,
                      const float* pad_val, int to_rgb, int seg_pad, int crop_h, int crop_w, float* img, uint8_t* masks, uint8_t* seg,
                      int32_t* stats, int H, int W, cgg_stream_t stream);

#define CGG_TRAIN_PREP_MAX_SEGMENTS 256
int cgg_train_prep_panoptic_u8(const uint8_t* staged, int64_t staged_bytes, int64_t img_table_offset, int64_t pan_table_offset,
                               int64_t seg_table_offset, const int32_t* img_table_host, const int32_t* pan_table_host,
                               const int32_t* seg_table_host, int B, int N, int S, const float* mean, const float* std,
                               const float* pad_val, int to_rgb, int seg_pad, int crop_h, int crop_w, float* img, uint8_t* masks,
                               uint8_t* seg, int32_t* stats, int H, int W, cgg_stream_t stream);

#define CGG_POLY_LDS_BITS 393216
#define CGG_POLY_SCAN_BITS 8192
int64_t cgg_train_prep_polygons_workspace_bytes(const int32_t* img_table_host, int B, int N, int force_workspace);
int cgg_polygon_fill_bits(const uint8_t* staged, int64_t staged_bytes, int64_t img_table_offset, int64_t inst_table_offset,
                          int64_t part_table_offset, const int32_t* img_table_host, const int32_t* inst_table_host,
                          const int32_t* part_table_host, const uint8_t* staged_host, int B, int N, int P, uint32_t* workspace,
                          int64_t workspace_bytes, int force_workspace, cgg_stream_t stream);
int cgg_train_prep_polygons_u8(const uint8_t* staged, int64_t staged_bytes, int64_t img_table_offset, int64_t inst_table_offset,
                               int64_t part_table_offset, const int32_t* img_table_host, const int32_t* inst_table_host,
                               const int32_t* part_table_host, const uint8_t* staged_host, int B, int N, int P, const float* mean,
                               const float* std, const float* pad_val, int to_rgb, int crop_h, int crop_w, float* img,
                               uint8_t* masks, int32_t* stats, int H, int W, uint32_t* workspace, int64_t workspace_bytes,
                               int force_workspace, cgg_stream_t stream);

#define CGG_BEAM_STEP_MAX_BEAM 8
#define CGG_BEAM_STEP_MAX_LEN 256
int64_t cgg_beam_step_workspace_bytes(int B, int beam, int V);
int cgg_beam_step(const float* logits, int L, int B, int beam, int V, int32_t* seqs, float* weights, int32_t* nlive,
                  int32_t* fin_seqs, int32_t* fin_len, float* fin_score, int32_t* nfin, int32_t* best_idx, int32_t* done,
                  int32_t* ndone, int64_t* tokens, int64_t* parents, void* ws, int length, float alpha, int eos, int max_len,
                  int state_max_len, int first, cgg_stream_t stream);
int cgg_beam_step_passes(const float* logits, int L, int B, int beam, int V, int32_t* seqs, float* weights, int32_t* nlive,
                         int32_t* fin_seqs, int32_t* fin_len, float* fin_score, int32_t* nfin, int32_t* best_idx, int32_t* done,
                         int32_t* ndone, int64_t* tokens, int64_t* parents, void* ws, int length, float alpha, int eos,
                         int max_len, int state_max_len, int first, int passes, cgg_stream_t stream);

int cgg_transpose_f32(const float* in, float* out, int B, int R, int C, cgg_stream_t stream);
int cgg_nchw_to_nhwc_pad1_f32(const float* in, float* out, int B, int C, int H, int W, cgg_stream_t stream);

int64_t cgg_wgrad_x3_workspace_bytes(int M, int N, int K);
int cgg_wgrad_x3(const float* dy, int ldy, const float* x, int ldx, float* ws, int* splits_out, int M, int N, int K,
                 cgg_stream_t stream);
int cgg_wgrad_bias_x3(const float* dy, int ldy, const float* x, int ldx, float* ws, float* ws_bias, int* splits_out, int M, int N,
                      int K, cgg_stream_t stream);

int cgg_topk_select(const float* x, int ld, int rows, int N, int k, int64_t* idx, cgg_stream_t stream);

int cgg_absmax_f32(const float* x, int ld, int M, int N, float* amax, cgg_stream_t stream);
int cgg_relu_bwd_absmax_f32(const float* gy, const float* y, float* g, long long n, float* amax, cgg_stream_t stream);
int cgg_gemm_x3_bwd(const float* a, int lda, const float* a_amax, const void* w_x3, const float* mask, int ldm, float* out, int ldc,
                    float* out_amax, int M, int N, int K, cgg_stream_t stream);
int cgg_gemm_x3_scaled(const float* a, int lda, const float* a_amax, const void* w_x3, const float* bias, const float* res, int ldr,
                       float* out, int ldc, int M, int N, int K, int relu, cgg_stream_t stream);
int cgg_conv_x3_nhwc_scaled(const float* x, const float* x_amax, const void* w_x3, const float* bias, const float* res, float* out,
                            int B, int H, int W, int C, int N, int KH, int KW, int stride, int pad, int relu, cgg_stream_t stream);
int cgg_wgrad_x3_scaled(const float* dy, int ldy, const float* dy_amax, const float* x, int ldx, float* ws, float* ws_bias,
                        int* splits_out, int M, int N, int K, cgg_stream_t stream);

int cgg_add_layernorm_ex(const void* a, int a_dtype, const void* b, int b_dtype, const float* gamma, const float* beta,
                         const float* pos, int pos_rows, float* y32, void* y16, void* yp16, int rows, int N,
                         float eps, cgg_stream_t stream);

int64_t cgg_add_layernorm_backward_partials(int rows);
int cgg_add_layernorm_backward(const float* dy, const void* dy16a, const void* dy16b, const float* a, const void* b, int b_dtype,
                               const float* gamma, float eps, float* dx, void* dx16, float* partial, int rows, int N,
                               cgg_stream_t stream);
int cgg_add_layernorm_backward_amax(const float* dy, const void* dy16a, const void* dy16b, const float* a, const void* b, int b_dtype,
                                    const float* gamma, float eps, float* dx, void* dx16, float* partial, float* dx_amax, int rows,
                                    int N, cgg_stream_t stream);

int cgg_encoder_proj_pack(const float* w, void* packed, int N, int K, cgg_stream_t stream);
int cgg_encoder_proj_bf16(const void* x16, const void* xp16, const void* pos16, int pos_rows, const void* wv_packed,
                          const float* bv, const void* wc_packed, const float* bc, void* value, void* offs, int M, int C, int NV,
                          int NC, int value_head_major_rows, cgg_stream_t stream);

int cgg_decoder_kv_pack_k(const float* w, void* packed, int N, int K, cgg_stream_t stream);
int cgg_decoder_kv_proj_bf16(const void* m16, const void* mp16, const void* wk_packed, const float* bk, const void* wv_packed,
                             void* k, void* vt, int B, int hw, int C, int NK, cgg_stream_t stream);

int cgg_bottleneck64_bf16(const void* x, const void* w1_packed, const float* b1, const void* w2_packed, const float* b2,
                          const void* w3_packed, const float* b3, void* y, int B, int H, int W, int C, int CMID, cgg_stream_t stream);

int cgg_encoder_ffn_ln_bf16(const void* x16, const void* w1_packed, const float* b1, const void* w2_packed,
                            const float* b2, const float* gamma, const float* beta, float eps, const float* pos,
                            int pos_rows, void* y16, void* yp16, float* y32, int M, int C, int F, cgg_stream_t stream);
int cgg_encoder_ffn_ln_kv_bf16(const void* x16, const void* w1_packed, const float* b1, const void* w2_packed,
                               const float* b2, const float* gamma, const float* beta, float eps, const float* shift,
                               const float* pos, int S, const int* level_start_host, int n_levels, float* y32, void* m16,
                               void* mp16, int M, int C, int F, cgg_stream_t stream);
int cgg_encoder_layer_tail_bf16(const void* a16, const void* x16, const void* wo_packed, const float* bo, const float* gamma0,
                                const float* beta0, float eps0, const void* w1_packed, const float* b1, const void* w2_packed,
                                const float* b2, const float* gamma1, const float* beta1, float eps1, const float* pos,
                                int pos_rows, const float* shift, const int* level_start_host, int n_levels, void* y16,
                                void* yp16, float* y32, int M, int C, int F, cgg_stream_t stream);

int cgg_add_layernorm_kv(const void* a, int a_dtype, const void* b, int b_dtype, const float* gamma, const float* beta,
                         const float* shift, const float* pos, int S, const int* level_start_host, int n_levels,
                         float* y32, void* m16, void* mp16, int rows, int N, float eps, cgg_stream_t stream);

int64_t cgg_group_norm_nhwc_workspace_bytes(int B, int HW, int groups);
int cgg_group_norm_nhwc(const void* x, const float* gamma, const float* beta, void* ws, int B, int HW, int C,
                        int groups, float eps, int relu, const float* up_src, int up_h, int up_w,
                        int64_t up_bstride, int W, float* y32, int64_t y32_bstride, void* y16, const float* pos,
                        void* yp16, int64_t y16_bstride, cgg_stream_t stream);
int cgg_pack_mask_feature_nhwc(const void* feat, void* hi, int B, int C, int H, int W, int pool,
                               cgg_stream_t stream);
int cgg_pack_mask_feature_nhwc_multi(const void* feat, void* const* hi_host, const int* pools_host, int n, int B, int C,
                                     int H, int W, cgg_stream_t stream);

// ... 105 lines not shown
```

Measured before the change: 420.5 images/sec.

## Compact residual tables with column windows and per-row broadcast in x3s GEMM

Adds a column-window residual mode to the x3s GEMM epilogue. Only the columns that vary per row (MSDA offsets/weights, K position bias) are read from a compact table, and the constant columns (value bias) come from a single broadcast row vector, so the zero and broadcast parts of the full-width table are no longer stored or read. It also adds an optional image-interleaved tile ordering so tiles sharing the same residual rows run close together, which should help cache reuse. The cost is more epilogue branching and template instantiations, plus extra validation paths.

```diff
diff --git a/betrayed-by-captions_amd/csrc/x3s_gemm.hip b/betrayed-by-captions_amd/csrc/x3s_gemm.hip
--- a/betrayed-by-captions_amd/csrc/x3s_gemm.hip
+++ b/betrayed-by-captions_amd/csrc/x3s_gemm.hip
@@ -16,6 +16,9 @@
   const float* bias;
   const void* res;
   int ldr, res_fmt, res_mod;
+  int res_cperiod, res_c0, res_cw, res_w;
+  const float* res_row;
+  int img_b, img_tiles;
   void* out;
   int ldc, out_fmt;
   int M, N, K, relu, tiles_n, n_tiles32;
@@ -57,11 +60,17 @@
   return r;
 }
 
+__device__ __forceinline__ int xs_res_col(const XsArgs& p, int ncol0) {
+  if (!p.res_cperiod) return ncol0;
+  const int k = ncol0 / p.res_cperiod, c = ncol0 - k * p.res_cperiod - p.res_c0;
+  return (unsigned)c < (unsigned)p.res_cw ? k * p.res_cw + c : -1;
+}
+
 __device__ __forceinline__ void xs_load_res(u32x4 (&rv)[4], const XsArgs& p, const __amdgpu_buffer_rsrc_t rrsrc, int& mres, int ncol0,
-                                            int lane) {
+                                            int tcol0, int lane) {
   const int q = lane & 7;
   const bool cok = ncol0 + 4 * q < p.N;
-  const uint32_t coff = (uint32_t)(ncol0 * 4 + 16 * q);
+  const uint32_t coff = (uint32_t)(tcol0 * 4 + 16 * q);
 #pragma unroll
   for (int ps = 0; ps < 4; ++ps) {
     int mr = mres + 8 * ps;
@@ -77,15 +86,19 @@
 
 template <int RES, int OUT, int TW = 0>
 __device__ __forceinline__ float xs_finish_column(const float* scratch, int TM_, const XsArgs& p, const XsEpi& e, int mrow0, int ncol0,
-                                                  int lane, float amax, const u32x4 (&rv0)[4], bool have_rv0) {
+                                                  int tcol0, int lane, float amax, const u32x4 (&rv0)[4], bool have_rv0) {
+  constexpr bool TAB = RES == 1 || RES == 2;
   const int r8 = lane >> 3, q = lane & 7;
   const uint32_t om = 0u - (uint32_t)(q & 1);
   const bool cok = ncol0 + 4 * q < p.N;
   const uint32_t coff = (uint32_t)(ncol0 * 4 + 16 * q);
   int mres = e.mr0;
-  auto load_res = [&](u32x4 (&rv)[4]) { xs_load_res(rv, p, e.rrsrc, mres, ncol0, lane); };
+  auto load_res = [&](u32x4 (&rv)[4]) { xs_load_res(rv, p, e.rrsrc, mres, ncol0, tcol0, lane); };
   u32x4 rv[4], rn[4];
-  if (RES) {
+  f32x4 rowv = {0.f, 0.f, 0.f, 0.f};
+  if (RES == 3)
+    rowv = *reinterpret_cast<const f32x4*>(p.res_row + (cok ? ncol0 + 4 * q : 0)) * CGG_X3_ASCALE;
+  if (TAB) {
     if (have_rv0) {
 #pragma unroll
       for (int ps = 0; ps < 4; ++ps) rv[ps] = rv0[ps];
@@ -98,7 +111,7 @@
 #pragma unroll 1
   for (int mt = 0; mt < TM_; ++mt) {
     const float* sc = scratch + mt * 1024;
-    if (RES && mt + 1 < TM_) load_res(rn);
+    if (TAB && mt + 1 < TM_) load_res(rn);
     f32x4 v[4];
 #pragma unroll
     for (int ps = 0; ps < 4; ++ps) {
@@ -123,6 +136,8 @@
         const f32x2 l0 = __builtin_convertvector(__builtin_bit_cast(f16x2, ll.x), f32x2);
         const f32x2 l1 = __builtin_convertvector(__builtin_bit_cast(f16x2, ll.y), f32x2);
         w += f32x4{h0[0] + l0[0], h0[1] + l0[1], h1[0] + l1[0], h1[1] + l1[1]};
+      } else if (RES == 3) {
+        w += rowv;
       }
 #pragma unroll
       for (int k = 0; k < 4; ++k) w[k] = fmaxf(w[k], e.lo_clamp);
@@ -147,7 +162,7 @@
       }
       __builtin_amdgcn_raw_buffer_store_b128(o, e.orsrc, oo, 0, 0);
     }
-    if (RES) {
+    if (TAB) {
 #pragma unroll
       for (int ps = 0; ps < 4; ++ps) rv[ps] = rn[ps];
     }
@@ -159,14 +174,14 @@
   XsEpi e;
   e.orsrc = cgg_buffer_rsrc(p.out, (uint32_t)(((size_t)(p.M - 1) * p.ldc + p.N) * 4));
   const int res_rows = p.res_mod ? p.res_mod : p.M;
-  e.rrsrc = cgg_buffer_rsrc(p.res_fmt ? p.res : p.out, p.res_fmt ? (uint32_t)(((size_t)(res_rows - 1) * p.ldr + p.N) * 4) : 0u);
+  e.rrsrc = cgg_buffer_rsrc(p.res_fmt ? p.res : p.out, p.res_fmt ? (uint32_t)(((size_t)(res_rows - 1) * p.ldr + p.res_w) * 4) : 0u);
   e.lo_clamp = p.relu ? 0.f : -__builtin_inff();
   e.mr0 = mrow0 + (lane >> 3);
   if (p.res_fmt && p.res_mod) e.mr0 %= p.res_mod;
   return e;
 }
 
-template <int TM, int TN, int TW = 0>
+template <int TM, int TN, int TW = 0, bool WIN = false>
 __device__ __forceinline__ float xs_epilogue(const f32x16 (&acc)[TM][TN], float* scratch, const XsArgs& p, const XsEpi& e, int mrow0,
                                              int ntile0, int lane, const u32x4 (&rv0)[4]) {
   const int j = lane & 31, hi5 = lane >> 5;
@@ -188,16 +203,23 @@
     }
     const int ncol0 = (ntile0 + nt) * 32;
     if constexpr (TW > 0) {
-      amax = fmt == 0 ? xs_finish_column<0, 1, TW>(scratch, TM, p, e, mrow0, ncol0, lane, amax, rv0, false)
-                      : xs_finish_column<0, 2, TW>(scratch, TM, p, e, mrow0, ncol0, lane, amax, rv0, false);
-    } else
-    switch (fmt) {
-      case 0: amax = xs_finish_column<0, 1>(scratch, TM, p, e, mrow0, ncol0, lane, amax, rv0, false); break;
-      case 1: amax = xs_finish_column<0, 2>(scratch, TM, p, e, mrow0, ncol0, lane, amax, rv0, false); break;
-      case 2: amax = xs_finish_column<1, 1>(scratch, TM, p, e, mrow0, ncol0, lane, amax, rv0, nt == 0); break;
-      case 3: amax = xs_finish_column<1, 2>(scratch, TM, p, e, mrow0, ncol0, lane, amax, rv0, nt == 0); break;
-      case 4: amax = xs_finish_column<2, 1>(scratch, TM, p, e, mrow0, ncol0, lane, amax, rv0, nt == 0); break;
-      default: amax = xs_finish_column<2, 2>(scratch, TM, p, e, mrow0, ncol0, lane, amax, rv0, nt == 0); break;
+      amax = fmt == 0 ? xs_finish_column<0, 1, TW>(scratch, TM, p, e, mrow0, ncol0, ncol0, lane, amax, rv0, false)
+                      : xs_finish_column<0, 2, TW>(scratch, TM, p, e, mrow0, ncol0, ncol0, lane, amax, rv0, false);
+    } else {
+      const int tcol0 = WIN ? xs_res_col(p, ncol0) : ncol0;
+      const int f = tcol0 >= 0 ? fmt : (p.res_row ? 6 : 0) + (p.out_fmt - 1);
+      switch (f) {
+        case 0: amax = xs_finish_column<0, 1>(scratch, TM, p, e, mrow0, ncol0, ncol0, lane, amax, rv0, false); break;
+        case 1: amax = xs_finish_column<0, 2>(scratch, TM, p, e, mrow0, ncol0, ncol0, lane, amax, rv0, false); break;
+        case 2: amax = xs_finish_column<1, 1>(scratch, TM, p, e, mrow0, ncol0, tcol0, lane, amax, rv0, nt == 0); break;
+        case 3: amax = xs_finish_column<1, 2>(scratch, TM, p, e, mrow0, ncol0, tcol0, lane, amax, rv0, nt == 0); break;
+        case 4: amax = xs_finish_column<2, 1>(scratch, TM, p, e, mrow0, ncol0, tcol0, lane, amax, rv0, nt == 0); break;
+        default:
+          if (!WIN || f == 5) amax = xs_finish_column<2, 2>(scratch, TM, p, e, mrow0, ncol0, tcol0, lane, amax, rv0, nt == 0);
+          else if (f == 6) amax = xs_finish_column<3, 1>(scratch, TM, p, e, mrow0, ncol0, ncol0, lane, amax, rv0, false);
+          else amax = xs_finish_column<3, 2>(scratch, TM, p, e, mrow0, ncol0, ncol0, lane, amax, rv0, false);
+          break;
+      }
     }
   }
   return amax;
@@ -269,7 +291,10 @@
   const int kg = wave / NWG, wg = wave - kg * NWG;
   const int wm = wg / WN, wn = wg - wm * WN;
   const int bid = cgg_xcd_remap(blockIdx.x, gridDim.x);
-  const int tile_m = bid / p.tiles_n, tile_n = bid - tile_m * p.tiles_n;
+  int tile_m = bid / p.tiles_n;
+  const int tile_n = bid - tile_m * p.tiles_n;
+  if constexpr (!CONV)
+    if (p.img_b > 1) tile_m = (tile_m % p.img_b) * p.img_tiles + tile_m / p.img_b;
   const int m0 = tile_m * BM, nt0 = tile_n * (BN / 32);
   const int KS = p.K >> 4, nchunk = p.K >> 5;
   const int niter = (nchunk + KG - 1) / KG;
@@ -402,8 +427,9 @@
   const XsEpi epi = xs_epi_setup(p, m0 + wm * TM * 32, lane);
   u32x4 rv0[4];
   if (p.res_fmt && (KG == 1 || kg == 0)) {
+    const int ncol0 = (nt0 + wn * TN) * 32, tcol0 = CONV ? ncol0 : xs_res_col(p, ncol0);
     int mres = epi.mr0;
-    xs_load_res(rv0, p, epi.rrsrc, mres, (nt0 + wn * TN) * 32, lane);
+    if (tcol0 >= 0) xs_load_res(rv0, p, epi.rrsrc, mres, ncol0, tcol0, lane);
   }
   int a_rd = 0, b_rd = 0;
   for (int it = 0; it < niter; ++it) {
@@ -445,7 +471,7 @@
   }
 
   float* scratch = reinterpret_cast<float*>(xs_smem + (KG - 1) * NWG * TM * TN * 4096 + wg * (TM * 4096));
-  const float amax = xs_epilogue<TM, TN>(acc, scratch, p, epi, m0 + wm * TM * 32, nt0 + wn * TN, lane, rv0);
+  const float amax = xs_epilogue<TM, TN, 0, !CONV>(acc, scratch, p, epi, m0 + wm * TM * 32, nt0 + wn * TN, lane, rv0);
   if (p.out_fmt == 2 && p.flag && !(amax <= CGG_X3A_MAX)) atomicOr(p.flag, 1);
 }
 
@@ -626,6 +652,9 @@
   CGG_RAISE_LDS((cgg_gemm_x3s_kernel<CONV, TM, TN, WM, WN, KG, SA, SB>), LDS, who);
   XsArgs b = a;
   b.tiles_n = (a.N + BN - 1) / BN;
+  const int imgs = (!CONV && a.img_b && a.res_mod > 0 && a.M % a.res_mod == 0 && a.res_mod % BM == 0) ? a.M / a.res_mod : 0;
+  b.img_b = imgs >= 2 ? imgs : 0;
+  b.img_tiles = b.img_b ? a.res_mod / BM : 0;
   const dim3 grid((unsigned)(((a.M + BM - 1) / BM) * b.tiles_n)), block(64 * WM * WN * KG);
   hipLaunchKernelGGL((cgg_gemm_x3s_kernel<CONV, TM, TN, WM, WN, KG, SA, SB>), grid, block, LDS, stream, b);
   return CGG_OK;
@@ -681,10 +710,31 @@
   return deep ? 12 : 13;
 }
 
+struct XsResCols {
+  int cperiod, c0, cw;
+  const float* row;
+  int img_order;
+};
+
 static int xs_launch(bool conv, const char* who, const void* a, int lda, const void* w_x3, const float* bias, const void* res, int ldr,
                      int res_fmt, int res_mod, void* out, int ldc, int out_fmt, int M, int N, int K, int relu, const XsConv& cv,
-                     cgg_stream_t stream, int a_rpb = 0, int64_t a_bstride = 0, int force_cfg = -1) {
+                     cgg_stream_t stream, int a_rpb = 0, int64_t a_bstride = 0, int force_cfg = -1, const XsResCols* xr = nullptr) {
   CGG_REQUIRE(a && w_x3 && out, CGG_EINVAL, "%s: null pointer", who);
+  int res_w = N;
+  if (xr && (xr->cperiod || xr->c0 || xr->cw || xr->row)) {
+    CGG_REQUIRE(xr->cperiod > 0 && xr->c0 >= 0 && xr->cw > 0 && xr->c0 + xr->cw <= xr->cperiod, CGG_EINVAL,
+                "%s: bad residual column window (period %d, first %d, width %d; res_row needs a window)", who, xr->cperiod, xr->c0,
+                xr->cw);
+    CGG_REQUIRE(xr->cperiod % 32 == 0 && xr->c0 % 32 == 0 && xr->cw % 32 == 0, CGG_EUNSUPPORTED,
+                "%s: residual column window (period %d, first %d, width %d) must be multiples of 32", who, xr->cperiod, xr->c0,
+                xr->cw);
+    CGG_REQUIRE(N % xr->cperiod == 0 || N < xr->cperiod, CGG_EUNSUPPORTED,
+                "%s: N=%d must be a multiple of the residual column period %d (or smaller)", who, N, xr->cperiod);
+    CGG_REQUIRE(res && res_fmt == 1 && res_mod > 0, CGG_EUNSUPPORTED,
+                "%s: a residual column window needs a row-periodic f32 residual (res_fmt %d, res_mod %d)", who, res_fmt, res_mod);
+    CGG_REQUIRE(cgg_aligned16(xr->row), CGG_EALIGN, "%s: res_row must be 16-byte aligned", who);
+    res_w = (N >= xr->cperiod ? N / xr->cperiod : 1) * xr->cw;
+  }
   CGG_REQUIRE(a_rpb >= 0 && (a_rpb == 0 || (!conv && a_bstride >= (int64_t)(a_rpb - 1) * lda + K && a_bstride % 8 == 0)), CGG_EINVAL,
               "%s: bad batched A (rows per image %d, image stride %lld)", who, a_rpb, (long long)a_bstride);
   CGG_REQUIRE(M > 0 && N > 0 && K > 0, CGG_EINVAL, "%s: bad sizes", who);
@@ -695,14 +745,14 @@
   CGG_REQUIRE(cgg_aligned16(a) && cgg_aligned16(w_x3) && cgg_aligned16(out) && cgg_aligned16(res) && (conv || lda % 8 == 0) &&
                   ldc % 8 == 0 && (!res || ldr % 8 == 0),
               CGG_EALIGN, "%s: pointers must be 16-byte aligned, row strides multiples of 8 (lda=%d ldc=%d ldr=%d)", who, lda, ldc, ldr);
-  CGG_REQUIRE(!res || ldr >= N, CGG_EINVAL, "%s: ldr=%d < N", who, ldr);
+  CGG_REQUIRE(!res || ldr >= res_w, CGG_EINVAL, "%s: ldr=%d < the residual's %d columns", who, ldr, res_w);
   CGG_REQUIRE(ldc >= N, CGG_EINVAL, "%s: ldc=%d < N", who, ldc);
   CGG_REQUIRE(res_mod >= 0 && (!res_mod || res), CGG_EINVAL, "%s: res_mod without res", who);
   CGG_REQUIRE(!conv || (cv.taps >= 1 && cv.taps <= 32), CGG_EUNSUPPORTED, "%s: at most 32 filter taps", who);
   const uint64_t a_bytes = conv    ? (uint64_t)(M / (cv.OH * cv.OW)) * cv.H * cv.W * cv.C * 4
                            : a_rpb ? ((uint64_t)((M - 1) / a_rpb) * a_bstride + (uint64_t)((M - 1) % a_rpb) * lda + K) * 4
                                    : ((uint64_t)(M - 1) * lda + K) * 4;
-  const uint64_t o_bytes = ((uint64_t)(M - 1) * ldc + N) * 4, r_bytes = res ? ((uint64_t)((res_mod ? res_mod : M) - 1) * ldr + N) * 4 : 0;
+  const uint64_t o_bytes = ((uint64_t)(M - 1) * ldc + N) * 4, r_bytes = res ? ((uint64_t)((res_mod ? res_mod : M) - 1) * ldr + res_w) * 4 : 0;
   CGG_REQUIRE(a_bytes < 0xFFFFFF00ull && o_bytes < 0xFFFFFF00ull && r_bytes < 0xFFFFFF00ull, CGG_EUNSUPPORTED,
               "%s: an operand spans more than 4 GiB (a %llu, out %llu, res %llu bytes)", who, (unsigned long long)a_bytes,
               (unsigned long long)o_bytes, (unsigned long long)r_bytes);
@@ -717,6 +767,13 @@
   x.ldr = ldr;
   x.res_fmt = res_fmt;
   x.res_mod = res_mod;
+  x.res_cperiod = xr ? xr->cperiod : 0;
+  x.res_c0 = x.res_cperiod ? xr->c0 : 0;
+  x.res_cw = x.res_cperiod ? xr->cw : 0;
+  x.res_w = res_w;
+  x.res_row = x.res_cperiod ? xr->row : nullptr;
+  x.img_b = xr ? xr->img_order : 0;
+  x.img_tiles = 0;
   x.out = out;
   x.ldc = ldc;
   x.out_fmt = out_fmt;
@@ -783,6 +840,17 @@
                    cv, stream, rows_per_image, a_bstride);
 }
 
+extern "C" int cgg_gemm_x3s_res(const void* a_x3a, int lda, int rows_per_image, int64_t a_bstride, const void* w_x3, const float* bias,
+                                const void* res, int ldr, int res_fmt, int res_mod, int res_cperiod, int res_c0, int res_cw,
+                                const float* res_row, void* out, int ldc, int out_fmt, int M, int N, int K, int relu, int cfg,
+                                int img_order, cgg_stream_t stream) {
+  const XsConv cv = {0, 0, 0, 0, 0, 0, 0, 0, 0};
+  const XsResCols rc = {res_cperiod, res_c0, res_cw, res_row, img_order};
+  CGG_REQUIRE(lda >= K && rows_per_image >= 0, CGG_EINVAL, "cgg_gemm_x3s_res: lda=%d < K or rows_per_image=%d", lda, rows_per_image);
+  return xs_launch(false, "cgg_gemm_x3s_res", a_x3a, lda, w_x3, bias, res, ldr, res_fmt, res_mod, out, ldc, out_fmt, M, N, K, relu, cv,
+                   stream, rows_per_image, a_bstride, cfg, &rc);
+}
+
 static int xs_conv(const void* x_x3a, const void* w_x3, const float* bias, const void* res, int res_fmt, void* out, int out_fmt, int B,
                    int H, int W, int C, int N, int KH, int KW, int stride, int pad, int relu, int cfg, cgg_stream_t stream) {
   CGG_REQUIRE(B > 0 && H > 0 && W > 0 && C > 0 && KH > 0 && KW > 0 && stride > 0 && pad >= 0, CGG_EINVAL,
diff --git a/betrayed-by-captions_amd/mask2former_head.py b/betrayed-by-captions_amd/mask2former_head.py
--- a/betrayed-by-captions_amd/mask2former_head.py
+++ b/betrayed-by-captions_amd/mask2former_head.py
@@ -700,6 +700,29 @@
         return dict(stream=x3_stream, kvs=kvs, sizes=sizes, packed_full=packed_full, pooled=pooled,
                     mask_features=mask_features)
 
+    @staticmethod
+    def _compact_kv_ok(E):
+        return E % 32 == 0
+
+    def _kv_blocks_x3a(self, attns, pos, lvl, E):
+        le = self.level_embed.weight[lvl].double()
+        ws, kbs, vbs = [], [], []
+        for a in attns:
+            w_kv, b_kv = a.kv_weight()
+            wd, bd = w_kv.double(), b_kv.double()
+            kbs.append((pos.double() + le) @ wd[:E].t() + bd[:E])
+            vbs.append(le @ wd[E:].t() + bd[E:])
+            ws.append(w_kv.float())
+        return torch.cat(ws, 0).contiguous(), kbs, vbs
+
+    @staticmethod
+    def _kv_residual(kbs, vbs, compact):
+        if compact:
+            row = torch.cat([torch.cat([torch.zeros_like(vb), vb]) for vb in vbs]).float().contiguous()
+            return torch.cat(kbs, 1).float().contiguous(), row
+        tabs = [torch.cat([kb, vb.expand(kb.shape[0], vb.shape[0])], 1) for kb, vb in zip(kbs, vbs)]
+        return torch.cat(tabs, 1).float().contiguous(), None
+
     def _project_kv_x3a(self, memorys, sizes):
         layers = self.transformer_decoder.layers
         L, nl = self.num_transformer_feat_level, self.num_transformer_decoder_layers
@@ -713,22 +736,17 @@
             pos = self.decoder_positional_encoding.flat_unpadded(h, w, mem.device)
             E = attns[0].embed_dims
 
-            def make(attns=attns, pos=pos, lvl=lvl, E=E):
-                le = self.level_embed.weight[lvl].double()
-                ws, tabs = [], []
-                for a in attns:
-                    w_kv, b_kv = a.kv_weight()
-                    wd, bd = w_kv.double(), b_kv.double()
-                    kb = (pos.double() + le) @ wd[:E].t() + bd[:E]
-                    vb = (le @ wd[E:].t() + bd[E:]).expand(pos.shape[0], E)
-                    ws.append(w_kv.float())
-                    tabs.append(torch.cat([kb, vb], 1))
-                return ops.pack_linear_weight_x3(torch.cat(ws, 0).contiguous()), torch.cat(tabs, 1).float().contiguous()
+            compact = self._compact_kv_ok(E)
+
+            def make(attns=attns, pos=pos, lvl=lvl, E=E, compact=compact):
+                w_all, kbs, vbs = self._kv_blocks_x3a(attns, pos, lvl, E)
+                return (ops.pack_linear_weight_x3(w_all),) + self._kv_residual(kbs, vbs, compact)
 
             params = tuple(p for a in attns for p in (a.attn.in_proj_weight, a.attn.in_proj_bias)) + (self.level_embed.weight, pos)
-            wk, table = runtime.derived_cached('kv_stack_x3a', params, make)
-            nout = table.shape[1]
-            kv_all = ops.gemm_x3s(mem, wk, nout, None, res=table, res_mod=h * w).view(B, h * w, nout)
+            wk, table, row = runtime.derived_cached('kv_stack_x3a' if compact else 'kv_stack_x3a_full', params, make)
+            nout = len(attns) * 2 * E
+            kv_all = ops.gemm_x3s(mem, wk, nout, None, res=table, res_mod=h * w, res_cols=(2 * E, 0, E) if compact else None,
+                                  res_row=row).view(B, h * w, nout)
             for j, i in enumerate(idx):
                 kvs[i] = kv_all[:, :, j * 2 * E:(j + 1) * 2 * E]
         return kvs
diff --git a/betrayed-by-captions_amd/ops.py b/betrayed-by-captions_amd/ops.py
--- a/betrayed-by-captions_amd/ops.py
+++ b/betrayed-by-captions_amd/ops.py
@@ -1602,7 +1602,10 @@
     return X3A_SPLIT if split else X3A_F32
 
 
-def gemm_x3s(a, packed, N, bias=None, res=None, res_split=False, res_mod=0, relu=False, out=None, out_split=False, cfg=-1):
+def gemm_x3s(a, packed, N, bias=None, res=None, res_split=False, res_mod=0, relu=False, out=None, out_split=False, cfg=-1,
+             res_cols=None, res_row=None, img_order=True):
+    if res_cols is not None or res_row is not None:
+        return _gemm_x3s_res(a, packed, N, bias, res, res_split, res_mod, relu, out, out_split, cfg, res_cols, res_row, img_order)
     if a.dim() not in (2, 3) or a.stride(-1) != 1 or a.dtype != torch.float32 or not is_x3(packed):
         raise CggError('gemm_x3s: a must be a 2-D / 3-D float32-tagged tensor with a contiguous last dim, packed an x3 image')
     rpb, bstride = 0, 0
@@ -1627,6 +1630,48 @@
             _call('cgg_gemm_x3s_batched', pa, lda, rpb, bstride, *rest, stream_ptr(a.device))
         else:
             _call('cgg_gemm_x3s_cfg', pa, lda, *rest, int(cfg), stream_ptr(a.device))
+    return y
+
+
+def _gemm_x3s_res(a, packed, N, bias, res, res_split, res_mod, relu, out, out_split, cfg, res_cols, res_row, img_order):
+    if a.dim() not in (2, 3) or a.stride(-1) != 1 or a.dtype != torch.float32 or not is_x3(packed):
+        raise CggError('gemm_x3s: a must be a 2-D / 3-D float32-tagged tensor with a contiguous last dim, packed an x3 image')
+    rpb, bstride = 0, 0
+    if a.dim() == 3:
+        rpb, bstride = int(a.shape[1]), int(a.stride(0))
+        M, K, lda = a.shape[0] * a.shape[1], a.shape[2], int(a.stride(1))
+    else:
+        (M, K), lda = a.shape, int(a.stride(0))
+    _x3_check(packed, N, K, 'gemm_x3s')
+    if res_cols is None:
+        raise CggError('gemm_x3s: res_row needs res_cols, the column window it lies outside of')
+    try:
+        period, c0, cw = (int(v) for v in res_cols)
+    except (TypeError, ValueError):
+        raise CggError(f'gemm_x3s: res_cols must be (period, c0, cw), got {res_cols!r}') from None
+    if period <= 0 or c0 < 0 or cw <= 0 or c0 + cw > period:
+        raise CggError(f'gemm_x3s: res_cols {(period, c0, cw)}: 0 <= c0, 0 < cw and c0 + cw <= period expected')
+    if period % 32 or c0 % 32 or cw % 32 or (N % period and N > period):
+        raise CggError(f'gemm_x3s: res_cols {(period, c0, cw)} must be multiples of 32 and N={N} a multiple of the period (or '
+                       'smaller): the window is decided per 32-column tile')
+    if res is None or res_split or res_mod <= 0:
+        raise CggError('gemm_x3s: res_cols needs a row-periodic float32 `res` (res_mod > 0); the x3a residual form has no column '
+                       'window')
+    width = (N // period or 1) * cw
+    if res.dtype != torch.float32 or res.dim() != 2 or tuple(res.shape) != (res_mod, width) or not res.is_contiguous():
+        raise CggError(f'gemm_x3s: res must be a contiguous float32 ({res_mod}, {width}) table for res_cols {(period, c0, cw)}, got '
+                       f'{res.dtype} {tuple(res.shape)}')
+    if res_row is not None and (res_row.dtype != torch.float32 or tuple(res_row.shape) != (N,) or not res_row.is_contiguous()):
+        raise CggError(f'gemm_x3s: res_row must be a contiguous float32 ({N},) vector, got {res_row.dtype} {tuple(res_row.shape)}')
+    y = out if out is not None else torch.empty((M, N), dtype=torch.float32, device=a.device)
+    if y.dim() != 2 or y.stride(1) != 1 or y.shape != (M, N) or y.dtype != torch.float32:
+        raise CggError('gemm_x3s: bad `out` view')
+    with _timed('gemm_x3', flops=2.0 * M * N * K, bytes=4.0 * (M * K + M * N + res.numel() + (N if res_row is not None else 0)) +
+                4.0 * N * K, shape=(M, N, K)):
+        _call('cgg_gemm_x3s_res', dev_ptr(a, 'a', torch.float32, dense=False), lda, rpb, bstride, dev_ptr(packed),
+              dev_ptr(bias, 'bias', torch.float32), dev_ptr(res, 'res', torch.float32), width, X3A_F32, int(res_mod), period, c0, cw,
+              dev_ptr(res_row, 'res_row', torch.float32), dev_ptr(y, 'out', torch.float32, dense=False), y.stride(0),
+              _x3s_fmt(out_split), M, N, K, int(bool(relu)), int(cfg), int(bool(img_order)), stream_ptr(a.device))
     return y
 
 
diff --git a/betrayed-by-captions_amd/pixel_decoder.py b/betrayed-by-captions_amd/pixel_decoder.py
--- a/betrayed-by-captions_amd/pixel_decoder.py
+++ b/betrayed-by-captions_amd/pixel_decoder.py
@@ -781,8 +781,10 @@
                 b_all = runtime.derived_cached('msda_ball32', (vp.bias, so.bias, aw.bias),
                                                lambda: torch.cat([vp.bias, so.bias, aw.bias], 0).float().contiguous())
 
-                tab = self._proj_pos_table(layer, pos, so, aw, tuple(level_hw), N, C, n_cat)
-                rows_all = runtime.linear_x3s(src.view(B * N, C), w_all, b_all, res=tab, res_mod=N).view(B, N, C + n_cat)
+                compact = self._compact_proj_ok(C, n_cat)
+                tab = self._proj_pos_table(layer, pos, so, aw, tuple(level_hw), N, C, n_cat, compact=compact)
+                rows_all = runtime.linear_x3s(src.view(B * N, C), w_all, b_all, res=tab, res_mod=N,
+                                              res_cols=(C + n_cat, C, n_cat) if compact else None).view(B, N, C + n_cat)
                 a = ops.msda_forward_fused_rows(rows_all, level_hw, level_start, ref, attn.num_points, H, C // H)
                 src, srcp = ops.encoder_layer_tail_x3(a, src, x3w(attn.output_proj), attn.output_proj.bias,
                                                       (n0.weight, n0.bias, n0.eps), x3w(fc1), fc1.bias, x3w(fc2), fc2.bias,
@@ -802,10 +804,14 @@
                                                   (n1.weight, n1.bias, n1.eps), pos=pos, want_pos=not last, x3a=True)
         return src
 
-    def _proj_pos_table(self, layer, pos, so, aw, level_hw, N, C, n_cat):
+    @staticmethod
+    def _compact_proj_ok(C, n_cat):
+        return C % 32 == 0 and n_cat % 32 == 0
+
+    def _proj_pos_table(self, layer, pos, so, aw, level_hw, N, C, n_cat, compact=True):
         import collections
         cache = self.__dict__.setdefault('_proj_tables', collections.OrderedDict())
-        key = (id(layer), level_hw, str(pos.device))
+        key = (id(layer), level_hw, str(pos.device), bool(compact))
         ver = (so.weight._version, aw.weight._version, so.weight.data_ptr(), aw.weight.data_ptr(), self.level_encoding.weight._version)
         hit = cache.get(key)
         if hit is not None and hit[0] == ver:
@@ -813,8 +819,11 @@
             return runtime.keepalive(hit[1])
         with torch.no_grad():
             w_cat = torch.cat([so.weight, aw.weight], 0).float().contiguous()
-            t = torch.zeros((N, C + n_cat), dtype=torch.float32, device=pos.device)
-            t[:, C:] = runtime.linear_x3(pos.float().contiguous(), w_cat)
+            t = runtime.linear_x3(pos.float().contiguous(), w_cat).contiguous()
+            if not compact:
+                full = torch.zeros((N, C + n_cat), dtype=torch.float32, device=pos.device)
+                full[:, C:] = t
+                t = full
         cache[key] = (ver, t)
         while len(cache) > 2 * len(self.encoder.layers):
             cache.popitem(last=False)
@@ -827,7 +836,7 @@
         C, H = vp.weight.shape[1], attn.num_heads
         n_cat = so.weight.shape[0] + aw.weight.shape[0]
         return (MERGED_PROJ and H == 8 and C == 256 and vp.weight.shape[0] == 256 and attn.num_levels == 3 and attn.num_points == 4
-                and n_cat == 3 * H * attn.num_levels * attn.num_points and (C + n_cat) % 32 == 0
+                and n_cat == 3 * H * attn.num_levels * attn.num_points and C % 32 == 0 and n_cat % 32 == 0
                 and all(m.bias is not None for m in (vp, so, aw)))
 
     def _forward_stream_x3a(self, feats, defer_fpn=False, pack_pools=None):
diff --git a/betrayed-by-captions_amd/runtime.py b/betrayed-by-captions_amd/runtime.py
--- a/betrayed-by-captions_amd/runtime.py
+++ b/betrayed-by-captions_amd/runtime.py
@@ -838,13 +838,15 @@
             and weight.shape[1] % 32 == 0 and x.shape[-1] == weight.shape[1] and x.numel() // x.shape[-1] >= 512)
 
 
-def linear_x3s(x, weight, bias=None, res=None, res_split=False, res_mod=0, relu=False, out=None, out_split=False):
+def linear_x3s(x, weight, bias=None, res=None, res_split=False, res_mod=0, relu=False, out=None, out_split=False, res_cols=None,
+               res_row=None):
     from . import ops
     N, K = weight.shape
     x2 = x if x.dim() <= 3 else x.reshape(-1, K)
     wk = derived_cached('x3_image', (weight,), lambda: ops.pack_linear_weight_x3(weight))
     y = ops.gemm_x3s(x2, wk, N, bias.detach() if bias is not None else None, res=res, res_split=res_split, res_mod=res_mod,
-                     relu=relu, out=out.view(-1, N) if out is not None else None, out_split=out_split)
+                     relu=relu, out=out.view(-1, N) if out is not None else None, out_split=out_split, res_cols=res_cols,
+                     res_row=res_row)
     return out if out is not None else y.view(*x.shape[:-1], N)
 
 
diff --git a/include/cgg_hip.h b/include/cgg_hip.h
--- a/include/cgg_hip.h
+++ b/include/cgg_hip.h
@@ -252,6 +252,10 @@
 int cgg_gemm_x3s_batched(const void* a_x3a, int lda, int rows_per_image, int64_t a_bstride, const void* w_x3, const float* bias,
                          const void* res, int ldr, int res_fmt, int res_mod, void* out, int ldc, int out_fmt, int M, int N, int K,
                          int relu, cgg_stream_t stream);
+int cgg_gemm_x3s_res(const void* a_x3a, int lda, int rows_per_image, int64_t a_bstride, const void* w_x3, const float* bias,
+                     const void* res, int ldr, int res_fmt, int res_mod, int res_cperiod, int res_c0, int res_cw,
+                     const float* res_row, void* out, int ldc, int out_fmt, int M, int N, int K, int relu, int cfg, int img_order,
+                     cgg_stream_t stream);
 int cgg_conv_x3s_nhwc(const void* x_x3a, const void* w_x3, const float* bias, const void* res, int res_fmt, void* out,
                       int out_fmt, int B, int H, int W, int C, int N, int KH, int KW, int stride, int pad, int relu,
                       cgg_stream_t stream);
```

Measured after the change: 423.8 images/sec, median of 6. About the same (+0.8%).
